# mobeets/classifying-vae-lstm

Measured on AMD Instinct MI355X. Metric: piano-roll timesteps/sec (train), higher is better.
Workload: dtype f32; 1 GPU; cfg3: cl_vrnn batch 256/GPU x seq_len 128, latent 2, 10 classes, 88-dim piano-roll, Adam-WN, hipGraph=True; global_batch=256, seq_len=128, parallelism=dp1

## Files before the change

### classifying-vae-lstm_amd/_lib.py

```python
import ctypes as C
import os

_HERE = os.path.dirname(os.path.abspath(__file__))
LIB_PATH = os.environ.get("CLV_LIB") or os.path.join(_HERE, "libclvae_hip.so")

ABI_VERSION = 600
ACT_NONE, ACT_RELU, ACT_SIGMOID, ACT_MASKPOS = 0, 1, 2, 3
GATE_HARD_SIGMOID, GATE_SIGMOID = 0, 1

_f = C.c_float
_i = C.c_int
_p = C.c_void_p
_sz = C.c_size_t
_i64 = C.c_int64
_u64 = C.c_uint64
_u32 = C.c_uint32
_d = C.c_double


class VaeStepOpts(C.Structure):
    _fields_ = [("draw", _i), ("stream_w", _u32), ("stream_z", _u32), ("step", _u32),
                ("noise_seed", _u64), ("first_w", _u64), ("first_z", _u64),
                ("step_dev", _p), ("loss_means", _p), ("bump_iterations", _p), ("bf16", _i)]

# ... 56 lines not shown


class SkinnyProduct(C.Structure):
    _fields_ = [("A", C.c_void_p), ("lda", C.c_int), ("rows", C.c_int), ("B", C.c_void_p), ("ldb", C.c_int),
                ("N", C.c_int), ("K", C.c_int), ("C", C.c_void_p), ("ldc", C.c_int), ("bias_row", C.c_void_p)]


class LabelBwdRider(C.Structure):
    _fields_ = [("D", C.c_int), ("C", C.c_int), ("Kenc_w", C.c_void_p), ("Kdec_w", C.c_void_p), ("wargs", C.c_void_p),
                ("eps", C.c_void_p), ("onehot", C.c_void_p), ("W", C.c_void_p), ("hW", C.c_void_p), ("Ka", C.c_void_p),
                ("prior_logvar", C.c_float), ("class_weight", C.c_float), ("w_kl_weight", C.c_float), ("inv_b", C.c_float),
                ("dwargs", C.c_void_p), ("dhW", C.c_void_p), ("dKa", C.c_void_p), ("dba", C.c_void_p),
                ("ws", C.c_void_p), ("ws_bytes", C.c_size_t), ("job", C.c_void_p)]


class ProfRecord(C.Structure):
    _fields_ = [("name", C.c_char * 48), ("launches", C.c_int32), ("total_ms", C.c_float)]


def _args(kind, names):
    return [kind] * len(names.split())


_VRNN_GENERATE = _args(_i, "N S nsteps D H L C gate_act z_prior") + [_u64] + _args(_p, "x_seed w")
_VAE_GENERATE = _args(_i, "N nsteps D H L C use_x_prev z_prior") + [_u64] + _args(_p, "x_seed w")
_VARY = _args(_i, "N T D H L C gate_act|use_x_prev hist_source") + [_u64] + _args(_p, "sources x0 w_enc w_dec")
_DECODE = _args(_i, "N T D H L C gate_act|use_x_prev") + [_u64] + _args(_p, "z_in x0 history w_dec noise_rows")
_VRNN_ENC, _VRNN_DEC = _args(_p, "Kx_enc Kw_enc b_enc U_enc Wz bz"), _args(_p, "Kx_dec Kz Kw_dec b_dec U_dec Wo bo")
_VAE_ENC, _VAE_DEC = _args(_p, "Kh bh Kz bz"), _args(_p, "Kd bd Ko bo")
_TEMPER = [_p, _f, _f]
_OUT, _OUT_Z = _args(_p, "Xs xhat stream"), _args(_p, "Xs xhat zout stream")
_RESUME = [_u32] + _args(_p, "state_in state_out")

SIGNATURES = {
    "clv_version": (_i, []),
    "clv_device_count": (_i, []),
    "clv_error_string": (C.c_char_p, [_i]),
    "clv_gemm_auto_split": (_i, [_i, _i, _i]),
    "clv_gemm_workspace_bytes": (_sz, [_i, _i, _i]),
    "clv_gemm_f32": (_i, [_i, _i, _i, _i, _i, _f, _p, _i, _p, _i, _f, _p, _i, _p, _i, _p, _i, _p, _sz, _p, _p]),
    "clv_gemm_grouped_tn": (_i, [_p, _i, _i, _i, _p, _i, _f, _i, _p, _sz, _p, _p]),
    "clv_splitk_reduce_multi": (_i, [_p, _i, _p, _p, _p, _i, _p, _p, _i, _p]),
    "clv_splitk_reduce_multi_outer_supported": (_i, [_i, _i, _i, _i, _i]),
    "clv_splitk_reduce_multi_outer": (_i, [_p, _i, _p, _p, _p, _i, _p, _p, _i,
                                           _i, _i, _i, _p, _i, _i, _p, _i, _p, _i, _p, _p, _i, _p, _p, _p]),
    "clv_lstm_wgrad_supported": (_i, [_i, _i, _i, _i, _i]),
    "clv_lstm_wgrad_workspace_bytes": (_sz, [_i, _i, _i, _i, _i, _i]),
    "clv_lstm_wgrad_pair_supported": (_i, [_p, _p]),
    "clv_lstm_wgrad_pair_workspace_bytes": (_sz, [_i, _i, _i, _i, _i, _i]),
    "clv_lstm_wgrad_pair": (_i, [_p, _p, _i, _p, _p, _p]),
    "clv_lstm_wgrad": (_i, [_i, _i, _p, _i, _i, _i, _p, _i, _i, _i, _i, _p, _i, _i, _p, _i, _p, _i, _p, _i, _p, _i, _f,
                               _i, _p, _sz, _p, _p]),
    "clv_gemm_grouped_tn_small2": (_i, [_p, _i, _p, _p, _i, _p, _i, _i, _i, _p]),
    "clv_gemm_grouped_auto_split": (_i, [_p, _i, _i, _i]),
    "clv_gemm_grouped_workspace_bytes": (_sz, [_p, _i, _i, _i]),
    "clv_colsum_workspace_bytes": (_sz, [_i, _i]),
    "clv_colsum_f32": (_i, [_i, _i, _p, _i, _f, _p, _p, _sz, _p]),
    "clv_lstm_seq_fwd": (_i, [_i, _i, _i, _i, _p, _p, _p, _p, _p, _p, _p, _p, _p, _p, _p]),
    "clv_lstm_seq_bwd_z": (_i, [_i, _i, _i, _i, _p, _p, _p, _p, _p, _p, _p, _i, _p, _i, _p]),
    "clv_lstm_seq_bwd": (_i, [_i, _i, _i, _i, _p, _p, _p, _p, _p, _p, _p]),
    "clv_lstm_mx_supported": (_i, [_i, _i, _i, _i]),
    "clv_lstm_mx_fwd": (_i, [_i, _i, _i, _i, _p, _i, _i, _i, _p, _p, _i, _i, _p, _p, _p, _p, _p, _p, _p]),
    "clv_lstm_mx_bwd": (_i, [_i, _i, _i, _p, _p, _p, _p, _p, _p, _i, _p, _i, _p]),
    "clv_lstm_pair_supported": (_i, [_i, _i]),
    "clv_lstm_pair_pack_floats": (_sz, []),
    "clv_lstm_pair_pack": (_i, [_i, _i, _p, _p, _p, _p, _p, _p]),
    "clv_lstm_pair_fwd": (_i, [_i, _i, _i, _i, _i, _p, _p, _p, _i, _p, _p, _p, _p, _p, _p, _p, _p, _p, _p, _i, _p, _p, _p, _p, _p,
                               _p, _p]),
    "clv_lstm_pair_bwd": (_i, [_i, _i, _i, _i, _i, _f] + [_p] * 12 + [_p, _p, _p, _p, _sz, _p, _p, _p]),
    "clv_lstm_pair_bwd_workspace_bytes": (_sz, [_i, _i, _i]),
    "clv_sparse_proj_supported": (_i, [_i, _i]),
    "clv_sparse_proj_lds_bytes": (_sz, [_i, _i]),
    "clv_sparse_proj": (_i, [_i, _i, _i, _p, _i, _i, _p, _p, _i, _p]),
    "clv_sparse_proj2": (_i, [_i, _i, _i, _i, _i, _p, _i, _p, _p, _i, _p, _i, _p, _p, _p]),
    "clv_sparse_dense_supported": (_i, [_i]),
    "clv_sparse_dense": (_i, [_i, _i, _i, _p, _i, _p, _p, _i, _p, _i, _p]),
    "clv_sparse_outer": (_i, [_i, _i, _i, _p, _i, _p, _i, _p, _i, _p, _p, _i, _p, _p, _p]),
    "clv_dense_outer_bf16_supported": (_i, [_i, _i, _i, _i, _i]),
    "clv_dense_outer_bf16": (_i, [_i, _i, _i, _p, _i, _i, _p, _i, _p, _i, _p, _p, _i, _p, _p, _p]),
    "clv_gemm_bce_f32": (_i, [_i, _i, _i, _p, _i, _p, _i, _p, _p, _i, _f, _p, _p, _i, _p, _p]),
    "clv_out_head_train_supported": (_i, [_i, _i]),
    "clv_out_head_train_workspace_bytes": (_sz, [_i]),
    "clv_out_head_train": (_i, [_i, _i, _i, _p, _p, _p, _p, _i, _i, _f, _p, _p, _p, _p, _p, _p, _p, _sz, _p, _p]),
    "clv_latent_head_supported": (_i, [_i, _i]),
    "clv_latent_head_bwd_workspace_bytes": (_sz, [_i, _i]),
    "clv_latent_head_fwd": (_i, [_i, _i, _i, _p, _p, _p, _p, _p, _p, _i, _p, _p, _p]),
    "clv_latent_head_bwd": (_i, [_i, _i, _i, _p, _p, _p, _p, _p, _i, _f, _p, _p, _p, _p, _p, _sz, _p, _p]),
    "clv_vrnn_generate_supported": (_i, [_i, _i, _i, _i]),
    "clv_vrnn_generate": (_i, _VRNN_GENERATE + _VRNN_ENC + _VRNN_DEC + _OUT),
    "clv_vae_generate_supported": (_i, [_i, _i, _i, _i]),
    "clv_vae_generate": (_i, _VAE_GENERATE + _VAE_ENC + _VAE_DEC + _OUT),
    "clv_vrnn_generate_clamped": (_i, _VRNN_GENERATE + _VRNN_ENC + _VRNN_DEC + _args(_p, "clamp") + _OUT),
    "clv_vae_generate_clamped": (_i, _VAE_GENERATE + _VAE_ENC + _VAE_DEC + _args(_p, "clamp") + _OUT),
    "clv_vrnn_generate_tempered": (_i, _VRNN_GENERATE + _VRNN_ENC + _VRNN_DEC + _TEMPER + _OUT),
    "clv_vae_generate_tempered": (_i, _VAE_GENERATE + _VAE_ENC + _VAE_DEC + _TEMPER + _OUT),
    "clv_vrnn_vary": (_i, _VARY + _VRNN_ENC + _VRNN_DEC + _TEMPER + _OUT),
    "clv_vae_vary": (_i, _VARY + _VAE_ENC + _VAE_DEC + _TEMPER + _OUT),
    "clv_take_frame": (_i, [_i64, _i, _i, _p, _p, _p, _p]),
    "clv_vrnn_vary_latents": (_i, _VARY + _VRNN_ENC + _VRNN_DEC + _TEMPER + _OUT_Z),
    "clv_vae_vary_latents": (_i, _VARY + _VAE_ENC + _VAE_DEC + _TEMPER + _OUT_Z),
    "clv_vrnn_decode": (_i, _DECODE + _VRNN_DEC + _TEMPER[:2] + _OUT),
    "clv_vae_decode": (_i, _DECODE + _VAE_DEC + _TEMPER[:2] + _OUT),
    "clv_vrnn_generate_resume": (_i, _VRNN_GENERATE + _VRNN_ENC + _VRNN_DEC + _TEMPER + _RESUME + _OUT),
    "clv_vae_generate_resume": (_i, _VAE_GENERATE[:-2] + _args(_p, "w") + _VAE_ENC + _VAE_DEC + _TEMPER + _RESUME + _OUT),
    "clv_lerp_rows": (_i, [_i64, _i64] + [_p] * 7),
    "clv_sigmoid_temper": (_i, [_i64, _p, _f, _p]),
    "clv_scale_temper": (_i, [_i64, _p, _f, _p]),
    "clv_label_fwd": (_i, [_i, _i, _p, _p, _i, _p, _p, _f, _p, _p, _p]),
    "clv_label_bwd": (_i, [_i, _i, _p, _p, _i, _p, _p, _p, _p, _f, _f, _f, _f, _p, _p, _i, _p]),
    "clv_vae_fused_supported": (_i, [_i, _i, _i, _i, _i]),
    "clv_vae_fused_workspace_bytes": (_sz, [_i, _i, _i, _i, _i, _i, _i]),
    "clv_vae_fused_step": (_i, [_i, _i, _i, _i, _i, _i, _i, _p, _p, _p, _p, _p, _p, _p, _p, _p, C.c_long, _f, _f, _f, _f, _i,
                                _p, _p, _sz, _p, _p, _p, _p, _p, _p, _p, _p, _p]),
    "clv_vrnn_label_fwd": (_i, [_i, _i, _i, _i, _p, _p, _p, _p, _p, _f, _p, _p, _p, _p, _p, _p, _p, _p, _p, _p]),
    "clv_vrnn_label_fwd_x": (_i, [_i, _i, _i, _i, _p, _i, _i, _p, _p, _p, _p, _p, _p, _p, _p, _f, _p, _p, _p, _p, _p, _p, _p, _p, _p,
                                  _p, _p, _p, _p]),
    "clv_vrnn_label_fwd_x_proj_supported": (_i, [_i, _i, _i, _i, _i]),
    "clv_vrnn_label_fwd_parts": (_i, [_i, _i, _i, _i, _p, _i, _p, _p, _p, _p, _p, _p, _f, _p, _p, _p, _p, _p, _p, _p, _p, _p,
                                  _p, _p, _p]),
    "clv_dense_window_fwd_bf16_supported": (_i, [_i, _i, _i, _i, _i]),
    "clv_dense_window_fwd_bf16_splits": (_i, [_i, _i]),
    "clv_dense_window_fwd_bf16_workspace_bytes": (_sz, [_i, _i, _i]),
    "clv_dense_window_fwd_bf16": (_i, [_i, _i, _i, _p, _i, _i, _p, _i, _p, _sz, _p]),
    "clv_vrnn_label_bwd_workspace_bytes": (_sz, [_i, _i, _i]),
    "clv_vrnn_label_bwd": (_i, [_i, _i, _i, _i, _p, _p, _p, _p, _p, _p, _p, _p, _p, _p, _f, _f, _f, _f, _p, _p, _p, _p, _p, _sz,
                                   _p, _p]),
    "clv_gauss_fwd": (_i, [_i, _i, _p, _p, _p, _i, _p, _p]),
    "clv_gauss_bwd": (_i, [_i, _i, _p, _p, _p, _i, _f, _p, _p]),
    "clv_bernoulli_nll": (_i, [_i, _i, _p, _p, _i, _f, _p, _p, _p]),
    "clv_loss_sums": (_i, [_p, _i, _i, _p, _i, _i, _p, _i, _i, _p, _i, _i, _p, _i, _i, _p, _p]),
    "clv_sum_strided": (_i, [_i, _p, _i, _f, _p, _p]),
    "clv_act_grad": (_i, [_i64, _i, _p, _p, _p, _p]),
    "clv_axpy": (_i, [_i64, _f, _p, _p, _p]),
    "clv_gather_rows": (_i, [_i64, _i64, _p, _p, _p, _i64, _i64, _p]),
    "clv_adam_wn_plan_bytes": (_sz, [_p, _i]),
    "clv_adam_wn_plan_build": (_i, [_p, _i, _p]),
    "clv_adam_wn_workspace_bytes": (_sz, [_p, _i]),
    "clv_adam_wn_step": (_i, [_p, _i, _p, _p, _p, _p, _p, _p, _p, _p, _p, _i, _f, _f, _f, _f, _i, _p, _p, _sz, _p]),
    "clv_philox_normal2": (_i, [_p, _i64, _u32, _u64, _p, _i64, _u32, _u64, _u64, _u32, _p, _p]),
    "clv_gather_rows_multi": (_i, [_i64, _p, _i64, _i, _p, _p, _p, _p, _p, _p, _p, _p, _p, _p, _p, _p]),
    "clv_philox_normal": (_i, [_p, _i64, _u64, _u32, _p, _u32, _u64, _p]),
    "clv_philox_uniform": (_i, [_p, _i64, _u64, _u32, _p, _u32, _u64, _p]),
    "clv_i32_add": (_i, [_p, C.c_int32, _p]),
    "clv_iw_accumulate": (_i, [_i, _i, _i, _i, _p, _p, _p, _p, _p, _f, _i, _p, _p, _p]),
    "clv_iw_finish": (_i, [_i, _i, _i, _p, _p, _p, _p, _p]),
    "clv_smc_sample": (_i, [_i, _i, _i, _i, _i, _p, _p, _p, _p, _p, _p, _p, _p]),
    "clv_smc_resample": (_i, [_i, _i, _i, _i, _u64, _i64, _d] + [_p] * 9),
    "clv_smc_gather": (_i, [_i, _i, _i, _i, _i, _p, _p, _p, _p, _p, _p, _p]),
    "clv_smc_backtrack": (_i, [_i, _i, _i, _i, _i, _u64, _i64, _i, _p, _p, _p, _p, _p, _p]),
    "clv_smc_init_w": (_i, [_i, _i, _i, _i, _u64, _i64, _p, _p, _p, _p, _p]),
    "clv_smc_w_posterior": (_i, [_i, _i, _i, _i, _i, _p, _p, _p, _p, _p]),
    "clv_smc_take_w": (_i, [_i, _i, _i, _i, _p, _p, _p, _p]),
    "clv_key_track_windows": (_i, [_i, _i, _i, _i, _i, _i, _i, _p, _p, _p, _p, _p, _p, _p, _u64, _i64, _p, _p, _p]),
    "clv_key_track_smooth": (_i, [_i, _i, _p, _p, _p, _p, _d, _p, _p, _p, _p, _p]),
    "clv_bernoulli_sample": (_i, [_i64, _p, _p, _p, _p]),
    "clv_bernoulli_sample_clamped": (_i, [_i64, _i, _i, _i, _p, _p, _p, _p, _p, _p]),
    "clv_dropout_rows": (_i, [_i, _i, _i, _p, _i, _p, _i, _f, _f, _p, _i, _p]),
    "clv_graph_begin_capture": (_i, [_p]),
    "clv_graph_end_capture": (_i, [_p, C.POINTER(_p)]),
    "clv_graph_launch": (_i, [_p, _p]),
    "clv_graph_destroy": (_i, [_p]),
    "clv_prof_enable": (_i, [_i]),
    "clv_prof_collect": (_i, [C.POINTER(ProfRecord), _i]),
    "clv_prof_empty_scope": (_i, [_p]),
}

_lib = None


class ClvError(RuntimeError):
    pass


def lib():
    global _lib
    if _lib is None:
        if not os.path.exists(LIB_PATH):
            raise ClvError(
                "libclvae_hip.so is not built (%s). Run `python __graft_entry__.py` or "
                "`make -C classifying-vae-lstm_amd/csrc`. There is no CPU fallback." % LIB_PATH)
        import torch
        h = C.CDLL(LIB_PATH)
        for name, (res, args) in SIGNATURES.items():
            fn = getattr(h, name)
            fn.restype = res
            fn.argtypes = args
        if h.clv_version() != ABI_VERSION:
            raise ClvError("libclvae_hip.so has ABI version %d, this binding was written for %d (include/clvae.h: "
                           "CLV_ABI_VERSION); rebuild with `make -C classifying-vae-lstm_amd/csrc`"
                           % (h.clv_version(), ABI_VERSION))
        _lib = h
    return _lib


def require_gpu():
    n = lib().clv_device_count()
    if n <= 0:
        raise ClvError("no gfx950 (MI355X) device visible; the HIP path has no CPU fallback")
    return n


def check(code, what=""):
# ... 4 lines not shown
```

### classifying-vae-lstm_amd/csrc/label_head.hip

```cpp
#include "common.h"
#include "lstm_pair_pack.h"
#include "philox.h"
#include "reduce_job.h"
#include "label_bwd_row.h"

namespace clv {

struct LabelFwdArgs {
  int B, D, C, G4;
  const float* hW;
  __device__ float* hW_out() const { return const_cast<float*>(hW); }
  const float* Ka;
  const float* ba;
  float* eps;
  struct { int on; uint32_t k0, k1, stream, step; uint64_t first; const int32_t* step_dev; } noise;
  const float* onehot;
  float prior;
  const float* Kenc_w;
  const float* benc;
  const float* Kdec_w;
  const float* bdec;
  float* wargs;
  float* W;
  float* rowloss;
  float* rb_enc;
  float* rb_dec;
};

template <int NT>
__device__ __forceinline__ void label_fwd_row(const LabelFwdArgs& a, int b, int tid, const float* s_h, float* s_wargs, float* s_w,
                                              long long oh_row = -1) {
  const int C1 = a.C - 1, NA = 2 * C1;
  __shared__ float s_eps[LH_MAXC], s_oh[LH_MAXC];
  if (tid >= NT - 64 && tid - (NT - 64) < a.C) {
    const int j = tid - (NT - 64);
    float e = 0.f;
    if (j < C1) {
      if (a.noise.on) {
        e = philox_normal_at(a.noise.first + (uint64_t)b * C1 + j, a.noise.k0, a.noise.k1, a.noise.stream,
                             a.noise.step + (a.noise.step_dev ? (uint32_t)*a.noise.step_dev : 0u));
        a.eps[(size_t)b * C1 + j] = e;
      } else {
        e = a.eps[(size_t)b * C1 + j];
      }
    }
    s_eps[j] = e;
    s_oh[j] = a.onehot ? a.onehot[(size_t)(oh_row < 0 ? b : oh_row) * a.C + j] : 0.f;
  }
  {
    __shared__ float s_part[16][2 * LH_MAXC];
    constexpr int KSL = NT / 64 < 16 ? NT / 64 : 16;
    const int col = tid & 63, sl = tid >> 6;
    if (sl < KSL) {
      float kv[(128 + KSL - 1) / KSL];
      const int cc = min(col, NA - 1);
#pragma unroll
      for (int i = 0; i < (128 + KSL - 1) / KSL; ++i) kv[i] = a.Ka[(size_t)min(sl + KSL * i, a.D - 1) * NA + cc];
      float acc = 0.f;
#pragma unroll
      for (int i = 0; i < (128 + KSL - 1) / KSL; ++i) acc = fmaf(sl + KSL * i < a.D ? s_h[sl + KSL * i] : 0.f, kv[i], acc);
      if (col < NA) s_part[sl][col] = acc;
    }
    __syncthreads();
    if (tid < NA) {
      float acc = a.ba[tid];
#pragma unroll
      for (int i = 0; i < KSL; ++i) acc += s_part[i][tid];
      s_wargs[tid] = acc;
      a.wargs[(size_t)b * NA + tid] = acc;
    }
  }
  __syncthreads();
  if (tid == 0) {
    float e[LH_MAXC];
    float S = 1.f, klw = 0.f;
    const float ep = __expf(a.prior);
    for (int j = 0; j < C1; ++j) {
      const float m = s_wargs[j], lv = s_wargs[C1 + j];
      const float sd = expf(0.5f * lv);
      e[j] = expf(m + sd * s_eps[j]);
      S += e[j];
      klw += 1.f - a.prior + lv - sd * sd / ep - m * m / ep;
    }
    e[C1] = 1.f;
    const float invS = 1.f / S;
    float qs = 0.f, wbest = -1.f, tbest = -1.f;
    int amax = 0, tmax = 0;
    for (int j = 0; j < a.C; ++j) {
      const float w = e[j] * invS;
      s_w[j] = w;
      a.W[(size_t)b * a.C + j] = w;
      qs += w + LW2;
      if (w > wbest) { wbest = w; amax = j; }
      const float tj = s_oh[j];
      if (tj > tbest) { tbest = tj; tmax = j; }
    }
    float wrec = 0.f;
    if (a.onehot)
      for (int j = 0; j < a.C; ++j) {
        const float n = (s_w[j] + LW2) / qs;
        wrec -= s_oh[j] * logf(fminf(fmaxf(n, LEPS_K), 1.f - LEPS_K));
      }
    a.rowloss[(size_t)b * 3 + 0] = -0.5f * klw;
    a.rowloss[(size_t)b * 3 + 1] = (float)C1 * wrec;
    a.rowloss[(size_t)b * 3 + 2] = (a.onehot && amax == tmax) ? 1.f : 0.f;
  }
  __syncthreads();
  for (int c = tid; c < a.G4; c += NT) {
    float e = a.benc[c], d = a.bdec[c];
    for (int j0 = 0; j0 < a.C; j0 += 8) {
      float ke[8], kd[8];
#pragma unroll
      for (int q = 0; q < 8; ++q) {
        const int j = min(j0 + q, a.C - 1);
        ke[q] = a.Kenc_w[(size_t)j * a.G4 + c];
        kd[q] = a.Kdec_w[(size_t)j * a.G4 + c];
      }
#pragma unroll
      for (int q = 0; q < 8; ++q) {
        const float w = j0 + q < a.C ? s_w[j0 + q] : 0.f;
        e = fmaf(w, ke[q], e);
        d = fmaf(w, kd[q], d);
      }
    }
    a.rb_enc[(size_t)b * a.G4 + c] = e;
    a.rb_dec[(size_t)b * a.G4 + c] = d;
  }
}

__global__ __launch_bounds__(LH_T) void vrnn_label_fwd_kernel(LabelFwdArgs a) {
  __shared__ float s_h[128], s_wargs[2 * LH_MAXC], s_w[LH_MAXC];
  const int b = blockIdx.x, tid = threadIdx.x;
  if (tid < a.D) s_h[tid] = a.hW[(size_t)b * a.D + tid];
  __syncthreads();
  label_fwd_row<LH_T>(a, b, tid, s_h, s_wargs, s_w);
}

struct LabelFwdXArgs {
  LabelFwdArgs l;
  const float* X;
  const float* Kh;
  const float* bh;
  int nx, ldx;
  PairPackArgs pack;
  const float* part; int splits;
  struct Stage {
    int on;
    const unsigned char* cur; const unsigned char* hist;
    long long cur_stride, cur_offset, hist_stride, hist_offset, row0;
    const long long* cur_table; const long long* hist_table; const long long* idx;
    const int* step_dev; int step0, period; long long cur_s, cur_o;
    float* X; float* Xh; int hist_chunk; long long hist_ld;
    const float* w_src; float* w_out;
    unsigned char* X8; unsigned char* Xh8;
  } stage;
};
__device__ __forceinline__ void label_fwd_x_block(const LabelFwdXArgs& ax, const int b, float2 (*part)[64], float* s_h, float* s_wargs,
                                                  float* s_w) {
  const LabelFwdArgs& a = ax.l;
  const int tid = threadIdx.x, lane = tid & 63;
  if (ax.pack.out) {
    for (int i = b * 1024 + tid; i < PK_TOTAL; i += a.B * 1024)
      ax.pack.out[i] = pair_pack_element(i, ax.pack.L, ax.pack.U_e, ax.pack.U_d, ax.pack.Kz, ax.pack.Wz,
                                         [](const float* p) { return *p; });
  }
  const int wave = __builtin_amdgcn_readfirstlane(tid >> 6);
  const int n2 = a.D / 2;
  const int lc = min(lane, n2 - 1);
  const float2* K2 = reinterpret_cast<const float2*>(ax.Kh);
  const float* xr = ax.X + (size_t)b * ax.ldx;
  const unsigned char* xbytes = nullptr;
  long long oh_row = -1;
  if (ax.stage.on) {
    const LabelFwdXArgs::Stage& g = ax.stage;
    long long base = 0;
    if (g.step_dev) {
      int j = (*g.step_dev - g.step0) % g.period;
      j = j < 0 ? j + g.period : j;
      base = (long long)j * g.cur_s + g.cur_o;
    }
    const long long sr = g.idx ? g.idx[base + b] : g.row0 + base + b;
    oh_row = sr;
    xbytes = g.cur + (g.cur_table ? g.cur_table[sr] : sr) * g.cur_stride + g.cur_offset;
    const unsigned char* hb = g.hist ? g.hist + (g.hist_table ? g.hist_table[sr] : sr) * g.hist_stride + g.hist_offset : nullptr;
    if (g.X8) {
      unsigned* xo8 = reinterpret_cast<unsigned*>(g.X8 + (size_t)b * ax.nx);
      unsigned* ho8 = reinterpret_cast<unsigned*>(g.Xh8 + (size_t)b * ax.nx);
      for (int c = 4 * tid; c < ax.nx; c += 4 * 1024) {
        xo8[c >> 2] = *reinterpret_cast<const unsigned*>(xbytes + c);
        if (hb) ho8[c >> 2] = *reinterpret_cast<const unsigned*>(hb + c);
      }
    } else {
      float* xo = g.X + (size_t)b * ax.ldx;
      for (int c = 4 * tid; c < ax.nx; c += 4 * 1024) {
        const unsigned v = *reinterpret_cast<const unsigned*>(xbytes + c);
        *reinterpret_cast<float4*>(xo + c) = make_float4((float)(v & 255u), (float)((v >> 8) & 255u), (float)((v >> 16) & 255u), (float)(v >> 24));
      }
      if (hb) {
        const int pieces = ax.nx / g.hist_chunk;
        for (int c = 4 * tid; c < ax.nx; c += 4 * 1024) {
          const unsigned v = *reinterpret_cast<const unsigned*>(hb + c);
          const int p = c / g.hist_chunk, w = c - p * g.hist_chunk;
          *reinterpret_cast<float4*>(g.Xh + ((size_t)b * pieces + p) * g.hist_ld + w) =
              make_float4((float)(v & 255u), (float)((v >> 8) & 255u), (float)((v >> 16) & 255u), (float)(v >> 24));
        }
      }
    }
    if (g.w_out && tid < a.C) g.w_out[(size_t)b * a.C + tid] = g.w_src[(size_t)sr * a.C + tid];
  }
  float2 acc = make_float2(0.f, 0.f);
  const int nchunk = (ax.nx + 63) / 64;
  typedef const __attribute__((address_space(1))) unsigned* gwords;
  auto xload = [&](int ch) -> unsigned {
    const int i = min(min(ch, nchunk - 1) * 64 + lane, ax.nx - 1);
    return xbytes ? ((gwords)xbytes)[i >> 2] : __builtin_bit_cast(unsigned, xr[i]);
  };
  const int xsh = 8 * (lane & 3);
  auto xval = [&](unsigned raw) { return xbytes ? (float)((raw >> xsh) & 0xffu) : __builtin_bit_cast(float, raw); };
  unsigned xa = xload(wave), xb = xload(wave + 16);
  for (int ch = wave; ch < nchunk; ch += 32) {
    const float x0 = xval(xa), x1 = xval(xb);
    const int j0 = ch * 64, j1 = (ch + 16) * 64;
    xa = xload(ch + 32); xb = xload(ch + 48);
    unsigned long long m0 = __ballot(j0 + lane < ax.nx && x0 != 0.f);
    unsigned long long m1 = __ballot(ch + 16 < nchunk && j1 + lane < ax.nx && x1 != 0.f);
    while (m0 | m1) {
      int kk[8];
      float vv[8];
#pragma unroll
      for (int q = 0; q < 8; ++q) {
        unsigned long long& m = q < 4 ? m0 : m1;
        const bool on = m != 0;
        const int bit = on ? __builtin_ctzll(m) : 0;
        m = on ? (m & (m - 1)) : 0;
        kk[q] = (q < 4 ? j0 : j1) + bit;
        const float v = __builtin_bit_cast(float, __builtin_amdgcn_readlane(__builtin_bit_cast(int, q < 4 ? x0 : x1), bit));
        vv[q] = on ? v : 0.f;
      }
      float2 kr[8];
#pragma unroll
      for (int q = 0; q < 8; ++q) kr[q] = K2[(size_t)min(kk[q], ax.nx - 1) * n2 + lc];
#pragma unroll
      for (int q = 0; q < 8; ++q) { acc.x = fmaf(vv[q], kr[q].x, acc.x); acc.y = fmaf(vv[q], kr[q].y, acc.y); }
    }
  }
  part[wave][lane] = acc;
  __syncthreads();
  if (wave == 0 && lane < n2) {
    float2 t = make_float2(ax.bh[2 * lane], ax.bh[2 * lane + 1]);
#pragma unroll
    for (int w = 0; w < 16; ++w) { t.x += part[w][lane].x; t.y += part[w][lane].y; }
    t.x = fmaxf(t.x, 0.f); t.y = fmaxf(t.y, 0.f);
    s_h[2 * lane] = t.x; s_h[2 * lane + 1] = t.y;
    float* op = a.hW_out() + (size_t)b * a.D + 2 * lane;
    op[0] = t.x; op[1] = t.y;
  }
  __syncthreads();
  label_fwd_row<1024>(a, b, tid, s_h, s_wargs, s_w, oh_row);
}

__global__ __launch_bounds__(1024) void vrnn_label_fwd_x_kernel(LabelFwdXArgs ax) {
  __shared__ float2 part[16][64];
  __shared__ float s_h[128], s_wargs[2 * LH_MAXC], s_w[LH_MAXC];
  label_fwd_x_block(ax, (int)blockIdx.x, part, s_h, s_wargs, s_w);
}

constexpr int FP_RMAX = 64;
constexpr int FP_NC = 4;
#ifndef FP_PF
#define FP_PF 4
#endif
#ifndef FP_ROUND
#define FP_ROUND 1
#endif
#ifndef FP_ABL
#define FP_ABL 0
#endif
typedef unsigned u32x4_t __attribute__((ext_vector_type(4)));
struct FrameProjArgs {
  int T, N, ldo, wgs, nset;
  const float* K[2];
  float* out[2];
};

#ifdef FRONT_STAMPS
__device__ unsigned long long g_front_wg[2048][6];
#define FRONT_STAMP(k)                                                                                               \
  do {                                                                                                               \
    __syncthreads();                                                                                                 \
    if (threadIdx.x == 0 && blockIdx.x < 2048) {                                                                     \
      unsigned long long t__;                                                                                        \
      unsigned hw__, xcc__;                                                                                          \
      asm volatile("s_memrealtime %0\n\ts_waitcnt lgkmcnt(0)" : "=s"(t__));                                          \
      asm volatile("s_getreg_b32 %0, hwreg(HW_REG_HW_ID)" : "=s"(hw__));                                             \
      asm volatile("s_getreg_b32 %0, hwreg(HW_REG_XCC_ID)" : "=s"(xcc__));                                           \
      g_front_wg[blockIdx.x][k < 2 ? k : k + 2] = t__;                                                                \
      g_front_wg[blockIdx.x][2] = hw__; g_front_wg[blockIdx.x][3] = xcc__;                                           \
    }                                                                                                                \
  } while (0)
#else
#define FRONT_STAMP(k)
#endif

__device__ __forceinline__ void frame_proj_block(const LabelFwdXArgs& ax, const FrameProjArgs& fp, const int u, float* Kl,
                                                 const unsigned char** rowp) {
  const LabelFwdXArgs::Stage& g = ax.stage;
  const int tid = threadIdx.x, lane = tid & 63;
  const int wave = __builtin_amdgcn_readfirstlane(tid >> 6);
  const int grp = u / fp.wgs, w = u - grp * fp.wgs;
  const bool second = grp >= 2;
  const int nf = ax.l.D, B = ax.l.B;
  const int nch = fp.N / 2, c0 = (grp & 1) * nch;
  const float* K = second ? fp.K[1] : fp.K[0];
  float* out = second ? fp.out[1] : fp.out[0];
  {
    const int q4 = nch / 4, nv = nf * q4;
    float4* dst = reinterpret_cast<float4*>(Kl);
    for (int i0 = tid; i0 < nv; i0 += 4 * 1024) {
      float4 v[4];
#pragma unroll
      for (int q = 0; q < 4; ++q) {
        const int e = min(i0 + q * 1024, nv - 1), k = e / q4;
        v[q] = *reinterpret_cast<const float4*>(K + (size_t)k * fp.N + c0 + 4 * (e - k * q4));
      }
#pragma unroll
      for (int q = 0; q < 4; ++q)
        if (i0 + q * 1024 < nv) dst[i0 + q * 1024] = v[q];
    }
  }
  const int nrows = w < B ? (B - w + fp.wgs - 1) / fp.wgs : 0;
  if (tid < nrows) {
    const int b = w + tid * fp.wgs;
    long long base = 0;
    if (g.step_dev) {
      int j = (*g.step_dev - g.step0) % g.period;
      j = j < 0 ? j + g.period : j;
      base = (long long)j * g.cur_s + g.cur_o;
    }
    const long long sr = g.idx ? g.idx[base + b] : g.row0 + base + b;
    rowp[tid] = second ? g.hist + (g.hist_table ? g.hist_table[sr] : sr) * g.hist_stride + g.hist_offset
                       : g.cur + (g.cur_table ? g.cur_table[sr] : sr) * g.cur_stride + g.cur_offset;
  }
  __syncthreads();
  FRONT_STAMP(2);
  const int nq = nrows * fp.T;
  if (nq == 0) return;
  const int colb = min(lane, nch / 4 - 1) * 4;
// ... 19 lines not shown
  auto advance_a = [&]() {
    ta += 16;
    if (ta >= fp.T) {
      do { ta -= fp.T; ++ra; } while (ta >= fp.T);
      base_a = rowbase(ra);
    }
  };
  const unsigned so_step = 16u * (unsigned)fp.ldo * 4u, so_wrap = (unsigned)(fp.wgs - 1) * (unsigned)fp.T * (unsigned)fp.ldo * 4u;
  unsigned so = (unsigned)(((w + ri * fp.wgs) * fp.T + t) * fp.ldo + c0) * 4u;
  auto advance_c = [&]() {
    t += 16; so += so_step;
    while (t >= fp.T) { t -= fp.T; so += so_wrap; }
  };
  unsigned qx0[FP_PF], qx1[FP_PF];
#pragma unroll
  for (int j = 0; j < FP_PF; ++j) {
    const bool ok = wave + 16 * j < nq;
    frame(ok ? base_a : base0, ok ? ta : 0, qx0[j], qx1[j]);
    __builtin_amdgcn_raw_buffer_store_b128(u32x4_t{0u, 0u, 0u, 0u}, r_out, (int)0x80000000u, 0, 0);
    advance_a();
  }
  for (int qb = wave; qb < nq; qb += 16 * FP_PF) {
#pragma unroll
    for (int j = 0; j < FP_PF; ++j) {
      const int q = qb + 16 * j;
      const bool live = q < nq;
      const float fx0 = (float)((qx0[j] >> sh0) & 0xffu), fx1 = (float)((qx1[j] >> sh1) & 0xffu);
      const bool more = q + 16 * FP_PF < nq;
      if (FP_ABL != 3) frame(more ? base_a : base0, more ? ta : 0, qx0[j], qx1[j]);
      advance_a();
      unsigned long long m0 = __ballot(live && v0 && fx0 != 0.f), m1 = __ballot(live && v1 && fx1 != 0.f);
      float acc[FP_NC];
#pragma unroll
      for (int c = 0; c < FP_NC; ++c) acc[c] = 0.f;
      auto rounds = [&](unsigned long long m, const float fx, const int kbase) {
        if (FP_ROUND == 1) {
          while (m) {
            const int k = __builtin_ctzll(m);
            asm("s_bitset0_b64 %0, %1" : "+s"(m) : "s"(k));
            const float v = __builtin_bit_cast(float, __builtin_amdgcn_readlane(__builtin_bit_cast(int, fx), k));
            const float4 k4 = *reinterpret_cast<const float4*>(Kl + (kbase + k) * nch + colb);
            acc[0] = fmaf(v, k4.x, acc[0]); acc[1] = fmaf(v, k4.y, acc[1]); acc[2] = fmaf(v, k4.z, acc[2]); acc[3] = fmaf(v, k4.w, acc[3]);
          }
          return;
        }
        while (m) {
          float v[FP_ROUND], kv[FP_ROUND][FP_NC];
          bool on[FP_ROUND];
#pragma unroll
          for (int r = 0; r < FP_ROUND; ++r) {
            on[r] = m != 0;
            const int k = on[r] ? __builtin_ctzll(m) : 0;
            m &= m - 1;
            v[r] = __builtin_bit_cast(float, __builtin_amdgcn_readlane(__builtin_bit_cast(int, fx), k));
            const float4 k4 = *reinterpret_cast<const float4*>(Kl + (kbase + k) * nch + colb);
            kv[r][0] = k4.x; kv[r][1] = k4.y; kv[r][2] = k4.z; kv[r][3] = k4.w;
          }
#pragma unroll
          for (int r = 0; r < FP_ROUND; ++r)
#pragma unroll
            for (int c = 0; c < FP_NC; ++c) acc[c] = (r == 0 || on[r]) ? fmaf(v[r], kv[r][c], acc[c]) : acc[c];
        }
      };
      if (FP_ABL != 2) {
        rounds(m0, fx0, 0);
        rounds(m1, fx1, 64);
      } else {
        acc[0] = fx0; acc[1] = fx1;
      }
      __builtin_amdgcn_raw_buffer_store_b128(u32x4_t{__builtin_bit_cast(unsigned, acc[0]), __builtin_bit_cast(unsigned, acc[1]),
                                                      __builtin_bit_cast(unsigned, acc[2]), __builtin_bit_cast(unsigned, acc[3])},
                                             r_out, (int)((live && FP_ABL != 1) ? vo : 0x80000000u), (int)so, 0);
      advance_c();
    }
  }
}

__global__ __launch_bounds__(1024) __attribute__((amdgpu_num_sgpr(72))) void vrnn_front_kernel(LabelFwdXArgs ax, FrameProjArgs fp) {
  __shared__ float2 part[16][64];
  __shared__ float s_h[128], s_wargs[2 * LH_MAXC], s_w[LH_MAXC];
  __shared__ const unsigned char* rowp[FP_RMAX];
  extern __shared__ __attribute__((aligned(16))) float fp_kl[];
  FRONT_STAMP(0);
  if ((int)blockIdx.x < ax.l.B) label_fwd_x_block(ax, (int)blockIdx.x, part, s_h, s_wargs, s_w);
  else frame_proj_block(ax, fp, (int)blockIdx.x - ax.l.B, fp_kl, rowp);
  FRONT_STAMP(1);
}

__global__ __launch_bounds__(LH_T) void vrnn_label_fwd_parts_kernel(LabelFwdXArgs ax) {
  constexpr int NWV = LH_T / 64;
  __shared__ float2 part[NWV][64];
  __shared__ float s_h[128], s_wargs[2 * LH_MAXC], s_w[LH_MAXC];
  const LabelFwdArgs& a = ax.l;
  const int tid = threadIdx.x, lane = tid & 63;
  if (ax.pack.out) {
    for (int i = blockIdx.x * LH_T + tid; i < PK_TOTAL; i += gridDim.x * LH_T)
      ax.pack.out[i] = pair_pack_element(i, ax.pack.L, ax.pack.U_e, ax.pack.U_d, ax.pack.Kz, ax.pack.Wz,
                                         [](const float* p) { return *p; });
  }
  const int wave = __builtin_amdgcn_readfirstlane(tid >> 6);
  const int b = blockIdx.x;
  const int n2 = a.D / 2;
  const int lc = min(lane, n2 - 1);
  float2 acc = make_float2(0.f, 0.f);
  const float2* pp = reinterpret_cast<const float2*>(ax.part + (size_t)b * a.D) + lc;
  const size_t cs = (size_t)a.B * a.D / 2;
  for (int c0 = wave; c0 < ax.splits; c0 += 8 * NWV) {
    float2 v[8];
#pragma unroll
    for (int q = 0; q < 8; ++q) v[q] = pp[(size_t)min(c0 + NWV * q, ax.splits - 1) * cs];
#pragma unroll
    for (int q = 0; q < 8; ++q) {
      const float mk = c0 + NWV * q < ax.splits ? 1.f : 0.f;
      acc.x = fmaf(v[q].x, mk, acc.x); acc.y = fmaf(v[q].y, mk, acc.y);
    }
  }
  part[wave][lane] = acc;
  __syncthreads();
  if (wave == 0 && lane < n2) {
    float2 t = make_float2(ax.bh[2 * lane], ax.bh[2 * lane + 1]);
#pragma unroll
    for (int w = 0; w < NWV; ++w) { t.x += part[w][lane].x; t.y += part[w][lane].y; }
    t.x = fmaxf(t.x, 0.f); t.y = fmaxf(t.y, 0.f);
    s_h[2 * lane] = t.x; s_h[2 * lane + 1] = t.y;
    float* op = a.hW_out() + (size_t)b * a.D + 2 * lane;
    op[0] = t.x; op[1] = t.y;
  }
  __syncthreads();
  label_fwd_row<LH_T>(a, b, tid, s_h, s_wargs, s_w);
}

__global__ __launch_bounds__(LH_T) void vrnn_label_bwd_kernel(LabelBwdArgs a) {
  label_bwd_row<LH_T>(a, (int)blockIdx.x, (int)threadIdx.x);
}

}

using namespace clv;

extern "C" int clv_vrnn_label_fwd(int B, int D, int C, int G4, const float* hW, const float* Ka, const float* ba,
                                  const float* eps, const float* onehot, float prior_logvar,
                                  const float* Kenc_w, const float* benc, const float* Kdec_w, const float* bdec,
                                  float* wargs, float* W, float* rowloss, float* rb_enc, float* rb_dec, void* stream) {
  if (B <= 0 || D <= 0 || D > 128 || C < 2 || C > LH_MAXC || G4 <= 0) return CLV_EINVAL;
  if (!hW || !Ka || !ba || !eps || !Kenc_w || !benc || !Kdec_w || !bdec || !wargs || !W || !rowloss || !rb_enc || !rb_dec)
    return CLV_EINVAL;
  LabelFwdArgs a{B, D, C, G4, hW, Ka, ba, const_cast<float*>(eps), {0, 0, 0, 0, 0, 0, nullptr}, onehot, prior_logvar, Kenc_w, benc,
                 Kdec_w, bdec, wargs, W, rowloss, rb_enc, rb_dec};
  hipStream_t s = (hipStream_t)stream;
  ProfScope p("vrnn_label_fwd", s);
  hipLaunchKernelGGL(vrnn_label_fwd_kernel, dim3(B), dim3(LH_T), 0, s, a);
  return launch_status();
}

extern "C" size_t clv_vrnn_label_bwd_workspace_bytes(int B, int D, int C) {
  return (size_t)B * (D + 1) * 2 * (C - 1) * sizeof(float);
}

extern "C" int clv_vrnn_label_bwd(int B, int D, int C, int G4, const float* dzsum_enc, const float* dzsum_dec,
                                     const float* Kenc_w, const float* Kdec_w, const float* wargs, const float* eps,
                                     const float* onehot, const float* W, const float* hW, const float* Ka,
                                     float prior_logvar, float class_weight, float w_kl_weight, float inv_b,
                                     float* dwargs, float* dhW, float* dKa, float* dba, void* ws, size_t ws_bytes,
                                     clv_reduce_job* job, void* stream) {
  if (job) memset(job, 0, sizeof(*job));
  if (B <= 0 || D <= 0 || D > 128 || C < 2 || C > LH_MAXC || G4 <= 0) return CLV_EINVAL;
  if (!dzsum_enc || !dzsum_dec || !Kenc_w || !Kdec_w || !wargs || !eps || !onehot || !W || !hW || !Ka || !dwargs || !dhW)
    return CLV_EINVAL;
  const bool wg = dKa != nullptr;
  if (wg && (!dba || !ws || ws_bytes < clv_vrnn_label_bwd_workspace_bytes(B, D, C))) return CLV_EWORKSPACE;
  LabelBwdArgs a{B, D, C, G4, dzsum_enc, dzsum_dec, Kenc_w, Kdec_w, wargs, eps, onehot, W, hW, Ka,
                 prior_logvar, class_weight, w_kl_weight, inv_b, dwargs, dhW, wg ? (float*)ws : nullptr};
  hipStream_t s = (hipStream_t)stream;
  {
    ProfScope p("vrnn_label_bwd", s);
    hipLaunchKernelGGL(vrnn_label_bwd_kernel, dim3(B), dim3(LH_T), 0, s, a);
  }
  int st = launch_status();
  if (st || !wg) return st;
  ReduceJob j;
  memset(&j, 0, sizeof(j));
  const int NA = 2 * (C - 1);
  j.partial = (const float*)ws;
  j.M = D + 1; j.N = NA; j.splits = B; j.nprob = 2;
  j.alpha = 1.f; j.beta = 0.f; j.act = CLV_ACT_NONE;
  j.prob[0] = ReduceProb{dKa, NA, 0};
  j.prob[1] = ReduceProb{dba, NA, D};
  if (job && B > 1) memcpy(job, &j, sizeof(j));
  else st = launch_reduce(j, s);
  return st;
}

extern "C" int clv_vrnn_label_fwd_x_proj_supported(int B, int D, int nx, int T, int N);

static int label_fwd_x_launch(int B, int D, int C, int G4, const float* X, int ldx, int nx, const float* Kh, const float* part,
                              int splits, const clv_label_stage* stage, const float* bh, float* hW_out, const float* Ka, const float* ba,
                              float* eps, const float* onehot, float prior_logvar,
                              const float* Kenc_w, const float* benc, const float* Kdec_w, const float* bdec,
                              float* wargs, float* W, float* rowloss, float* rb_enc, float* rb_dec,
                              const clv_noise_draw* noise, const clv_pair_pack_src* pack, const clv_frame_proj* proj, void* stream) {
  if (pack && (pack->H != LH || !clv_lstm_pair_supported(pack->H, pack->L) || !pack->U_enc || !pack->U_dec || !pack->Kz ||
               !pack->Wz || !pack->pack || ((uintptr_t)pack->pack) % 16))
    return CLV_EINVAL;
  if (B <= 0 || D <= 0 || D > 128 || D % 2 != 0 || C < 2 || C > LH_MAXC || G4 <= 0) return CLV_EINVAL;
  if (part ? (splits <= 0 || ((uintptr_t)part) % 8 != 0)
           : (nx <= 0 || ldx < nx || (!X && !(stage && stage->X8)) || !Kh || ((uintptr_t)Kh) % 8 != 0)) return CLV_EINVAL;
  if (stage) {
    const clv_label_stage& g = *stage;
    if (part || !g.cur || nx % 4 || ldx % 4 || ((uintptr_t)g.cur) % 4 || g.cur_stride % 4 || g.cur_offset % 4) return CLV_EINVAL;
    if (g.hist && (((uintptr_t)g.hist) % 4 || g.hist_stride % 4 || g.hist_offset % 4)) return CLV_EINVAL;
    if (g.X8) {
      if (((uintptr_t)g.X8) % 4 || (g.hist && (!g.Xh8 || ((uintptr_t)g.Xh8) % 4))) return CLV_EINVAL;
    } else {
      if (!g.X || ((uintptr_t)g.X) % 16) return CLV_EINVAL;
      if (g.hist && (!g.Xh || g.hist_chunk <= 0 || g.hist_chunk % 4 || nx % g.hist_chunk || g.hist_ld % 4 || g.hist_ld < g.hist_chunk ||
                     ((uintptr_t)g.Xh) % 16))
        return CLV_EINVAL;
    }
    if ((g.w_out != nullptr) != (g.w_src != nullptr)) return CLV_EINVAL;
    if (g.cursor.step_dev && g.cursor.period < 1) return CLV_EINVAL;
  }
  if (!bh || !hW_out || !Ka || !ba || !eps || !Kenc_w || !benc || !Kdec_w || !bdec || !wargs || !W || !rowloss ||
      !rb_enc || !rb_dec)
    return CLV_EINVAL;
  LabelFwdXArgs a{{B, D, C, G4, hW_out, Ka, ba, eps, {0, 0, 0, 0, 0, 0, nullptr}, onehot, prior_logvar, Kenc_w, benc, Kdec_w, bdec,
                   wargs, W, rowloss, rb_enc, rb_dec}, X, Kh, bh, nx, ldx, {0, nullptr, nullptr, nullptr, nullptr, nullptr}, part, splits, {}};
  if (stage) {
    const clv_label_stage& g = *stage;
    a.stage = LabelFwdXArgs::Stage{1, g.cur, g.hist, (long long)g.cur_stride, (long long)g.cur_offset, (long long)g.hist_stride,
                                   (long long)g.hist_offset, (long long)g.row0, (const long long*)g.cur_table,
                                   (const long long*)g.hist_table, (const long long*)g.idx, g.cursor.step_dev, g.cursor.step0,
                                   g.cursor.period, (long long)g.cursor.stride, (long long)g.cursor.offset, g.X, g.Xh, g.hist_chunk,
                                   (long long)g.hist_ld, g.w_src, g.w_out, g.X8, g.Xh8};
    if (g.w_src) a.l.onehot = g.w_src;
  }
  if (pack) a.pack = PairPackArgs{pack->L, pack->U_enc, pack->U_dec, pack->Kz, pack->Wz, reinterpret_cast<float4*>(pack->pack)};
  if (noise) {
    a.l.noise.on = 1; a.l.noise.k0 = (uint32_t)noise->seed; a.l.noise.k1 = (uint32_t)(noise->seed >> 32);
    a.l.noise.stream = noise->stream; a.l.noise.step = noise->step; a.l.noise.first = noise->first;
    a.l.noise.step_dev = noise->step_dev;
  }
  hipStream_t s = (hipStream_t)stream;
  if (proj) {
    if (!clv_vrnn_label_fwd_x_proj_supported(B, D, nx, proj->T, proj->N) || !stage || !stage->X8 || part || proj->ldo < proj->N ||
        (size_t)B * proj->T * proj->ldo * 4 >= ((size_t)1 << 31) || proj->ldo % 4 || ((uintptr_t)proj->out_cur) % 16 || ((uintptr_t)proj->out_hist) % 16 ||
        !proj->K_cur || !proj->out_cur || ((uintptr_t)proj->K_cur) % 16 || (proj->K_hist && (!proj->out_hist || !stage->hist ||
        ((uintptr_t)proj->K_hist) % 16)))
      return CLV_EINVAL;
    FrameProjArgs fp;
    memset(&fp, 0, sizeof(fp));
    fp.T = proj->T; fp.N = proj->N; fp.ldo = proj->ldo; fp.nset = proj->K_hist ? 2 : 1;
    fp.K[0] = proj->K_cur; fp.out[0] = proj->out_cur; fp.K[1] = proj->K_hist; fp.out[1] = proj->out_hist;
    const int groups = 2 * fp.nset;
    int wgs = 256 / groups;
    wgs = wgs > B ? B : wgs;
    const int need = (B + FP_RMAX - 1) / FP_RMAX;
    wgs = wgs < need ? need : wgs;
    fp.wgs = wgs;
    size_t lds = (size_t)D * (proj->N / 2) * sizeof(float);
#ifdef FRONT_STAMPS
    if (const char* e = getenv("CLV_EXP_FRONT_LDS")) lds = (size_t)atoi(e);
#endif
    if (int e = clv::allow_dynamic_lds(reinterpret_cast<const void*>(vrnn_front_kernel), 64 * 1024)) return e;
    ProfScope p("vrnn_front", s);
    hipLaunchKernelGGL(vrnn_front_kernel, dim3(B + groups * wgs), dim3(1024), lds, s, a, fp);
    return launch_status();
  }
  ProfScope p("vrnn_label_fwd", s);
  if (part) hipLaunchKernelGGL(vrnn_label_fwd_parts_kernel, dim3(B), dim3(LH_T), 0, s, a);
  else hipLaunchKernelGGL(vrnn_label_fwd_x_kernel, dim3(B), dim3(1024), 0, s, a);
  return launch_status();
}

#ifdef FRONT_STAMPS
extern "C" int clv_debug_front_wg(unsigned long long* host_out) {
  return (int)hipMemcpyFromSymbol(host_out, HIP_SYMBOL(clv::g_front_wg), sizeof(unsigned long long) * 2048 * 6);
}
#endif

extern "C" int clv_vrnn_label_fwd_x_proj_supported(int B, int D, int nx, int T, int N) {
  return B >= 1 && D >= 4 && D <= 128 && D % 4 == 0 && T >= 1 && (long long)T * D == nx && N >= 8 && N % 8 == 0 && N / 2 <= 64 * clv::FP_NC &&
         (size_t)D * (N / 2) * sizeof(float) <= 64 * 1024 && (size_t)B * T * N * sizeof(float) < ((size_t)1 << 31);
}

extern "C" int clv_vrnn_label_fwd_x(int B, int D, int C, int G4, const float* X, int ldx, int nx, const float* Kh,
                                    const clv_label_stage* stage,
                                    const float* bh, float* hW_out, const float* Ka, const float* ba,
                                    float* eps, const float* onehot, float prior_logvar,
                                    const float* Kenc_w, const float* benc, const float* Kdec_w, const float* bdec,
                                    float* wargs, float* W, float* rowloss, float* rb_enc, float* rb_dec,
                                    const clv_noise_draw* noise, const clv_pair_pack_src* pack, const clv_frame_proj* proj,
                                    void* stream) {
  if (stage)
    return label_fwd_x_launch(B, D, C, G4, stage->X, ldx, nx, Kh, nullptr, 0, stage, bh, hW_out, Ka, ba, eps, stage->w_src,
                              prior_logvar, Kenc_w, benc, Kdec_w, bdec, wargs, W, rowloss, rb_enc, rb_dec, noise, pack, proj, stream);
  if (proj) return CLV_EINVAL;
  return label_fwd_x_launch(B, D, C, G4, X, ldx, nx, Kh, nullptr, 0, nullptr, bh, hW_out, Ka, ba, eps, onehot, prior_logvar, Kenc_w, benc,
                            Kdec_w, bdec, wargs, W, rowloss, rb_enc, rb_dec, noise, pack, nullptr, stream);
}

extern "C" int clv_vrnn_label_fwd_parts(int B, int D, int C, int G4, const float* part, int splits,
                                        const float* bh, float* hW_out, const float* Ka, const float* ba,
                                        float* eps, const float* onehot, float prior_logvar,
                                        const float* Kenc_w, const float* benc, const float* Kdec_w, const float* bdec,
                                        float* wargs, float* W, float* rowloss, float* rb_enc, float* rb_dec,
                                        const clv_noise_draw* noise, const clv_pair_pack_src* pack, void* stream) {
  if (!part) return CLV_EINVAL;
  return label_fwd_x_launch(B, D, C, G4, nullptr, 0, 0, nullptr, part, splits, nullptr, bh, hW_out, Ka, ba, eps, onehot, prior_logvar, Kenc_w,
                            benc, Kdec_w, bdec, wargs, W, rowloss, rb_enc, rb_dec, noise, pack, nullptr, stream);
}
```

### classifying-vae-lstm_amd/csrc/out_head.hip

```cpp
#include "out_head_args.h"
#include "reduce_job.h"

namespace clv {

typedef float f32x4 __attribute__((ext_vector_type(4)));

constexpr int OH_T = 6;
constexpr int OH_KS = OH / 4;
constexpr int OH_LD = 116;
constexpr int OH_NW = 8;
static_assert(OH_RB == 16 * OH_NW, "rows per block");
constexpr int OH_TILE = 16 * OH_LD;
constexpr int OH_P3 = 5;

#ifdef OH_STAMPS
__device__ unsigned long long g_oh_stamps[16];
#define OHS(k) do { if (blockIdx.x == 0 && threadIdx.x == 0) g_oh_stamps[k] = __builtin_readcyclecounter(); } while (0)
#else
#define OHS(k) do { } while (0)
#endif


__global__ __launch_bounds__(64 * OH_NW) void out_head_train_kernel(OutHeadArgs a) {
  extern __shared__ __attribute__((aligned(16))) float oh_lds[];
  float* WoL = oh_lds;
  float* hsT = oh_lds + OH * OH_LD;
  float* dlT = hsT + OH_NW * OH_TILE;
  const int tid = threadIdx.x, lane = tid & 63;
  const int wave = __builtin_amdgcn_readfirstlane(tid >> 6);
  const int r = lane & 15, q = lane >> 4;
  OHS(0);

  float bias[OH_T];
#pragma unroll
  for (int j = 0; j < OH_T; ++j) bias[j] = a.bo[min(16 * j + r, OH - 1)];

  const int t0 = wave < 4 ? OH_P3 * wave : 4 * OH_P3 + (OH_P3 - 1) * (wave - 4);
  const int nt = wave < 4 ? OH_P3 : OH_P3 - 1;
  int tm[OH_P3], tn[OH_P3];
  f32x4 acc3[OH_P3];
#pragma unroll
  for (int i = 0; i < OH_P3; ++i) {
    const int t = min(t0 + i, OH_T * OH_T - 1);
    tm[i] = t / OH_T; tn[i] = t - tm[i] * OH_T;
    acc3[i] = (f32x4){0.f, 0.f, 0.f, 0.f};
  }
  float* myhs = hsT + wave * OH_TILE;
  float* mydl = dlT + wave * OH_TILE;

  float4 hv[6];
  auto load_hs = [&](int row0) {
#pragma unroll
    for (int i = 0; i < 6; ++i) {
      const int e = min(lane + 64 * i, 16 * (OH / 4) - 1);
      const int rr = e / (OH / 4), c4 = e - rr * (OH / 4);
      hv[i] = *reinterpret_cast<const float4*>(a.hs + (size_t)min(row0 + rr, a.R - 1) * OH + 4 * c4);
    }
  };
  float y[OH_T][4];
  auto load_y = [&](int row0) {
#pragma unroll
    for (int j = 0; j < OH_T; ++j)
#pragma unroll
      for (int reg = 0; reg < 4; ++reg)
        y[j][reg] = static_cast<const float*>(a.Y)[(size_t)min(row0 + 4 * q + reg, a.R - 1) * a.ldy + min(16 * j + r, OH - 1)];
  };
  load_hs(blockIdx.x * OH_RB + wave * 16);
  load_y(blockIdx.x * OH_RB + wave * 16);
  {
    constexpr int NV = OH * (OH / 4);
    float4 wv[(NV + 64 * OH_NW - 1) / (64 * OH_NW)];
#pragma unroll
    for (int i = 0; i < (NV + 64 * OH_NW - 1) / (64 * OH_NW); ++i) {
      const int e = min(tid + 64 * OH_NW * i, NV - 1);
      const int h = e / (OH / 4), c4 = e - h * (OH / 4);
      wv[i] = *reinterpret_cast<const float4*>(a.Wo + h * OH + 4 * c4);
    }
#pragma unroll
    for (int i = 0; i < (NV + 64 * OH_NW - 1) / (64 * OH_NW); ++i) {
      const int e = tid + 64 * OH_NW * i;
      const int h = e / (OH / 4), c4 = e - h * (OH / 4);
      if (e < NV) *reinterpret_cast<float4*>(WoL + h * OH_LD + 4 * c4) = wv[i];
    }
// ... 102 lines not shown
#pragma unroll
          for (int j = 0; j < OH_T; ++j) bn[j] = WoL[wrow[j] + 4 * (s + 1)];
        }
        __builtin_amdgcn_sched_barrier(0);
#pragma unroll
        for (int j = 0; j < OH_T; ++j) acc[j] = __builtin_amdgcn_mfma_f32_16x16x4f32(av, bv[j], acc[j], 0, 0, 0);
        __builtin_amdgcn_sched_barrier(0);
        if (s + 1 < OH_KS) {
          av = an;
#pragma unroll
          for (int j = 0; j < OH_T; ++j) bv[j] = bn[j];
        }
      }
    }
#pragma unroll
    for (int reg = 0; reg < 4; ++reg) {
      const int row = row0 + 4 * q + reg;
#pragma unroll
      for (int j = 0; j < OH_T; ++j) {
        const int col = 16 * j + r;
        if (row < a.R && col < OH) a.dhs[(size_t)row * OH + col] = acc[j][reg];
      }
    }
    OHS(5);
    __syncthreads();
    OHS(6);

    {
      auto p3off = [&](int ks) { return (ks >> 2) * OH_TILE + ((ks & 3) * 4 + q) * OH_LD + r; };
      float av[OH_P3], bv[OH_P3];
#pragma unroll
      for (int i = 0; i < OH_P3; ++i) {
        av[i] = hsT[p3off(0) + 16 * tm[i]];
        bv[i] = dlT[p3off(0) + 16 * tn[i]];
      }
#pragma unroll 4
      for (int ks = 0; ks < OH_RB / 4; ++ks) {
        const int off = p3off(min(ks + 1, OH_RB / 4 - 1));
        float an[OH_P3], bn[OH_P3];
#pragma unroll
        for (int i = 0; i < OH_P3; ++i) {
          an[i] = hsT[off + 16 * tm[i]];
          bn[i] = dlT[off + 16 * tn[i]];
        }
        __builtin_amdgcn_sched_barrier(0);
#pragma unroll
        for (int i = 0; i < OH_P3; ++i)
          if (i < nt) acc3[i] = __builtin_amdgcn_mfma_f32_16x16x4f32(av[i], bv[i], acc3[i], 0, 0, 0);
        __builtin_amdgcn_sched_barrier(0);
#pragma unroll
        for (int i = 0; i < OH_P3; ++i) { av[i] = an[i]; bv[i] = bn[i]; }
      }
    }
    OHS(7);
    __syncthreads();
  }
  float* slab = a.partial + (size_t)blockIdx.x * OH_SLAB_ROWS * OH;
#pragma unroll
  for (int i = 0; i < OH_P3; ++i)
#pragma unroll
    for (int reg = 0; reg < 4; ++reg) {
      const int h = 16 * tm[i] + 4 * q + reg, o = 16 * tn[i] + r;
      if (i < nt && h < OH_SLAB_ROWS && o < OH) slab[h * OH + o] = acc3[i][reg];
    }
  OHS(8);
}

#ifdef OH_STAMPS
}
extern "C" int clv_debug_out_head_stamps(unsigned long long* host_out) {
  return (int)hipMemcpyFromSymbol(host_out, HIP_SYMBOL(clv::g_oh_stamps), sizeof(unsigned long long) * 16);
}
namespace clv {
#endif
static int out_head_wgs(int R) {
  const int blocks = (R + OH_RB - 1) / OH_RB;
  return blocks < 256 ? blocks : 256;
}

}

extern "C" int clv_out_head_train_supported(int H, int D) { return H == clv::OH && D == clv::OH; }

extern "C" size_t clv_out_head_train_workspace_bytes(int R) {
  return R > 0 ? (size_t)clv::out_head_wgs(R) * clv::OH_SLAB_ROWS * clv::OH * sizeof(float) : 0;
}

extern "C" int clv_out_head_train(int R, int H, int D, const float* hs, const float* Wo, const float* bo,
                                  const void* Y, int y_u8, int ldy, float scale, float* logits, float* rownll, float* dlogits,
                                  float* dhs, float* dWo, float* dbo, void* ws, size_t ws_bytes, clv_reduce_job* job,
                                  void* stream) {
  using namespace clv;
  if (!clv_out_head_train_supported(H, D) || R <= 0 || ldy < D) return CLV_EINVAL;
  if (!hs || !Wo || !bo || !Y || !rownll || !dhs || !dWo || !dbo) return CLV_EINVAL;
  if (((uintptr_t)hs) % 16 != 0 || ((uintptr_t)Wo) % 16 != 0) return CLV_EINVAL;
  if (!ws || ws_bytes < clv_out_head_train_workspace_bytes(R)) return CLV_EWORKSPACE;
  hipStream_t s = (hipStream_t)stream;
  const size_t lds = (size_t)(OH * OH_LD + 2 * OH_NW * OH_TILE) * sizeof(float);
  if (int e = clv::allow_dynamic_lds(reinterpret_cast<const void*>(out_head_train_kernel), (int)lds)) return e;
  const int wgs = out_head_wgs(R);
  OutHeadArgs a{R, ldy, scale, hs, Wo, bo, Y, y_u8 != 0, logits, rownll, dlogits, dhs, (float*)ws};
  static const bool f32_only = [] { const char* e = getenv("CLV_OUT_HEAD_F32"); return e && e[0] == '1'; }();
  if (!(f32_only && !y_u8) && out_head_bf16_ok(a)) {
    if (int e = launch_out_head_bf16(a, wgs, s)) return e;
  } else {
    if (y_u8) return CLV_EINVAL;
    ProfScope p("out_head_train", s);
    hipLaunchKernelGGL(out_head_train_kernel, dim3(wgs), dim3(64 * OH_NW), lds, s, a);
  }
  int st = launch_status();
  if (st) return st;
  ReduceJob j;
  memset(&j, 0, sizeof(j));
  j.partial = (const float*)ws; j.M = OH_SLAB_ROWS; j.N = OH; j.splits = wgs; j.nprob = 2;
  j.alpha = 1.f; j.beta = 0.f; j.act = CLV_ACT_NONE;
  j.prob[0] = ReduceProb{dWo, OH, 0};
  j.prob[1] = ReduceProb{dbo, OH, OH};
  if (job && wgs > 1) {
    memcpy(job, &j, sizeof(j));
    return CLV_OK;
  }
  if (job) memset(job, 0, sizeof(*job));
  return launch_reduce(j, s);
}
```

### classifying-vae-lstm_amd/csrc/out_head_args.h

```cpp
#pragma once
#include "common.h"

namespace clv {

constexpr int OH = 88;
constexpr int OH_SLAB_ROWS = OH + 1;
constexpr int OH_RB = 128;

struct OutHeadArgs {
  int R, ldy;
  float scale;
  const float* hs;
  const float* Wo;
  const float* bo;
  const void* Y;
  int y_u8;
  float* logits;
  float* rownll;
  float* dlogits;
  float* dhs;
  float* partial;
};

bool out_head_bf16_ok(const OutHeadArgs& a);
int launch_out_head_bf16(const OutHeadArgs& a, int wgs, hipStream_t s);

}
```

### classifying-vae-lstm_amd/csrc/out_head_bf16.hip

```cpp
#include "out_head_args.h"

namespace clv {

typedef __bf16 bf16x8 __attribute__((ext_vector_type(8)));
typedef float f32x4 __attribute__((ext_vector_type(4)));
typedef float f32x16 __attribute__((ext_vector_type(16)));
typedef unsigned u32x4 __attribute__((ext_vector_type(4)));

constexpr int OB_NW = 8;
constexpr int OB_FRAG = 1024;
constexpr int OB_IMG = 3 * 6 * 3 * OB_FRAG;
constexpr int OB_DLT = 96 * 16;
constexpr int OB_LDS = 2 * OB_IMG + OB_NW * OB_DLT * 4;
static_assert(OB_LDS <= 160 * 1024, "LDS");
static_assert(OB_NW * 18 * 64 * 16 <= OB_LDS, "the final reduction's rounds fit");

#ifdef OB_STAMPS
__device__ unsigned long long g_ob_stamps[16];
__device__ unsigned long long g_ob_wg[256][4];
#define OBW(k) do { if (threadIdx.x == 0) { unsigned long long t_; asm volatile("s_memrealtime %0\n\ts_waitcnt lgkmcnt(0)" : "=s"(t_)); g_ob_wg[blockIdx.x][k] = t_; } } while (0)
#define OBS(k) do { if (blockIdx.x == 0 && threadIdx.x == 0) g_ob_stamps[k] = __builtin_readcyclecounter(); } while (0)
#else
#define OBW(k) do { } while (0)
#define OBS(k) do { } while (0)
#endif

__device__ __forceinline__ void ob_split8(const float (&v)[8], u32x4 (&f)[3]) {
#pragma unroll
  for (int i = 0; i < 4; ++i) {
    unsigned pc[3];
#ifdef OB_SHIFT_SPLIT
    bf16_split_pair(v[2 * i], v[2 * i + 1], pc);
#else
    bf16_split_pair_dot2(v[2 * i], v[2 * i + 1], pc);
#endif
    f[0][i] = pc[0]; f[1][i] = pc[1]; f[2][i] = pc[2];
  }
}
__device__ __forceinline__ bf16x8 ob_frag(const u32x4& v) { return __builtin_bit_cast(bf16x8, v); }

typedef __amdgpu_buffer_rsrc_t ob_rsrc_t;
constexpr unsigned OB_OOB = 0x80000000u;
__device__ __forceinline__ ob_rsrc_t ob_rsrc(const void* p, size_t bytes) {
  return __builtin_amdgcn_make_buffer_rsrc(const_cast<void*>(p), 0, (int)(unsigned)bytes, 0x00020000);
}
__device__ __forceinline__ float ob_u2f(unsigned u) { return __builtin_bit_cast(float, u); }
__device__ __forceinline__ float ob_load1(ob_rsrc_t r, unsigned voff, int imm) {
  return __builtin_bit_cast(float, __builtin_amdgcn_raw_buffer_load_b32(r, (int)voff + imm, 0, 0));
}
__device__ __forceinline__ void ob_load4(ob_rsrc_t r, unsigned voff, float (&v)[4]) {
  const u32x4 x = __builtin_amdgcn_raw_buffer_load_b128(r, (int)voff, 0, 0);
#pragma unroll
  for (int i = 0; i < 4; ++i) v[i] = ob_u2f(x[i]);
}
__device__ __forceinline__ void ob_load8(ob_rsrc_t r, unsigned voff, float (&v)[8]) {
  const u32x4 x = __builtin_amdgcn_raw_buffer_load_b128(r, (int)voff, 0, 0);
  const u32x4 z = __builtin_amdgcn_raw_buffer_load_b128(r, (int)voff + 16, 0, 0);
#pragma unroll
  for (int i = 0; i < 4; ++i) { v[i] = ob_u2f(x[i]); v[4 + i] = ob_u2f(z[i]); }
}
__device__ __forceinline__ void ob_store4(const float (&v)[4], ob_rsrc_t r, unsigned voff) {
  const u32x4 x = {__builtin_bit_cast(unsigned, v[0]), __builtin_bit_cast(unsigned, v[1]), __builtin_bit_cast(unsigned, v[2]),
                   __builtin_bit_cast(unsigned, v[3])};
  __builtin_amdgcn_raw_buffer_store_b128(x, r, (int)voff, 0, 0);
}
__device__ __forceinline__ void ob_store1(float v, ob_rsrc_t r, unsigned voff) {
  __builtin_amdgcn_raw_buffer_store_b32(__builtin_bit_cast(unsigned, v), r, (int)voff, 0, 0);
}

#define OB_PROD6(MFMA, acc, A, B)                                   \
  do {                                                              \
    acc = MFMA(ob_frag(A[2]), ob_frag(B[0]), acc, 0, 0, 0);         \
    acc = MFMA(ob_frag(A[1]), ob_frag(B[1]), acc, 0, 0, 0);         \
    acc = MFMA(ob_frag(A[0]), ob_frag(B[2]), acc, 0, 0, 0);         \
    acc = MFMA(ob_frag(A[1]), ob_frag(B[0]), acc, 0, 0, 0);         \
    acc = MFMA(ob_frag(A[0]), ob_frag(B[1]), acc, 0, 0, 0);         \
    acc = MFMA(ob_frag(A[0]), ob_frag(B[0]), acc, 0, 0, 0);         \
  } while (0)

__device__ __forceinline__ int ob_dlt_line(int note) { return (((note >> 4) * 4 + (note & 3)) * 4 + ((note >> 2) & 3)) * 16; }

template <bool YU8>
__global__ __launch_bounds__(64 * OB_NW) void out_head_bf16_kernel(OutHeadArgs a) {
  extern __shared__ __attribute__((aligned(16))) char ob_lds[];
  char* A1 = ob_lds;
  char* A2 = ob_lds + OB_IMG;
  const int tid = threadIdx.x, lane = tid & 63;
  const int wave = __builtin_amdgcn_readfirstlane(tid >> 6);
  const int r = lane & 15, q = lane >> 4, n32 = lane & 31, kh = lane >> 5;
  float* dlT = reinterpret_cast<float*>(ob_lds + 2 * OB_IMG) + wave * OB_DLT;
  OBS(0);
  OBW(0);

  const ob_rsrc_t r_hs = ob_rsrc(a.hs, (size_t)a.R * OH * 4), r_y = ob_rsrc(a.Y, (size_t)a.R * a.ldy * (YU8 ? 1 : 4));
  const ob_rsrc_t r_lg = ob_rsrc(a.logits, a.logits ? (size_t)a.R * OH * 4 : 0);
  const ob_rsrc_t r_dl = ob_rsrc(a.dlogits, a.dlogits ? (size_t)a.R * OH * 4 : 0);
  const ob_rsrc_t r_dh = ob_rsrc(a.dhs, (size_t)a.R * OH * 4), r_nl = ob_rsrc(a.rownll, (size_t)a.R * 4);
  const unsigned c_off = (16 * 0 + 4 * q) * 4u;
  const bool c5 = q < 2;

  float hv[3][8];
  auto load_hv = [&](int row0) {
#pragma unroll
    for (int s = 0; s < 3; ++s)
      ob_load8(r_hs, (s == 2 && q == 3) ? OB_OOB : (unsigned)(row0 + r) * (OH * 4u) + (32 * s + 8 * q) * 4u, hv[s]);
  };
  load_hv(blockIdx.x * OH_RB + wave * 16);

  {
    const ob_rsrc_t r_wo = ob_rsrc(a.Wo, (size_t)OH * OH * 4), r_bo = ob_rsrc(a.bo, (size_t)OH * 4);
    const int m = r, qq = q;
    const unsigned l0 = (8 * qq * OH + m) * 4u;
    const unsigned l1 = (m * OH + 4 * qq) * 4u;
    float wv[5][8];
#pragma unroll
    for (int it = 0; it < 5; ++it) {
      const int F = min(8 * it + wave, 35);
      const int img = F >= 18, fr = F - 18 * img, j = fr / 3, s = fr - 3 * j;
      if (!img) {
        const unsigned vo = (16 * j + m < OH) ? l0 + (32 * s * OH + 16 * j) * 4u : OB_OOB;
#pragma unroll
        for (int e = 0; e < 8; ++e) wv[it][e] = ob_u2f(__builtin_amdgcn_raw_buffer_load_b32(r_wo, (int)vo + e * OH * 4, 0, 0));
        const float bias = ob_u2f(__builtin_amdgcn_raw_buffer_load_b32(r_bo, (s == 2 && qq == 3) ? (16 * j + m) * 4 : (int)OB_OOB, 0, 0));
        wv[it][0] = (s == 2 && qq == 3) ? bias : wv[it][0];
      } else {
        const unsigned vo = l1 + (16 * j * OH + 32 * s) * 4u;
        const u32x4 lo = __builtin_amdgcn_raw_buffer_load_b128(r_wo, (int)vo, 0, 0);
        const u32x4 hi = __builtin_amdgcn_raw_buffer_load_b128(r_wo, (s == 2 && qq >= 2) ? (int)OB_OOB : (int)vo + 64, 0, 0);
#pragma unroll
        for (int e = 0; e < 4; ++e) { wv[it][e] = ob_u2f(lo[e]); wv[it][4 + e] = ob_u2f(hi[e]); }
      }
    }
#pragma unroll
    for (int it = 0; it < 5; ++it) {
      const int F = 8 * it + wave;
      if (F < 36) {
        u32x4 f[3];
        ob_split8(wv[it], f);
        char* base = (F >= 18 ? A2 + (F - 18) * OB_FRAG : A1 + F * OB_FRAG) + lane * 16;
#pragma unroll
        for (int p = 0; p < 3; ++p) *reinterpret_cast<u32x4*>(base + p * 18 * OB_FRAG) = f[p];
      }
    }
  }

  f32x16 acc3[3][3];
#pragma unroll
  for (int i = 0; i < 3; ++i)
#pragma unroll
    for (int j = 0; j < 3; ++j)
#pragma unroll
      for (int e = 0; e < 16; ++e) acc3[i][j][e] = 0.f;
#pragma unroll
  for (int s = 0; s < 3; ++s) asm volatile("" :: "v"(hv[s][0]), "v"(hv[s][4]));
  OBS(10);
  __syncthreads();
  OBS(1);
  OBW(1);

  for (int blk = blockIdx.x; blk * OH_RB < a.R; blk += gridDim.x) {
    const int row0 = blk * OH_RB + wave * 16;
    if (row0 >= a.R) continue;
    const unsigned row = row0 + r;
    const bool rok = (int)row < a.R;
    const unsigned o_row = row * (OH * 4u) + c_off;
    const unsigned o5 = c5 ? o_row + 5 * 64 : OB_OOB;

    load_hv(row0);
    OBS(2);

    float y[6][4];
    f32x4 acc[6];
#pragma unroll
    for (int j = 0; j < 6; ++j) acc[j] = (f32x4){0.f, 0.f, 0.f, 0.f};
#pragma unroll
    for (int s = 0; s < 3; ++s) {
      if (s == 2) hv[2][0] = q == 3 ? 1.f : hv[2][0];
      u32x4 B[3];
      ob_split8(hv[s], B);
      if (s == 2) {
        __builtin_amdgcn_sched_barrier(0);
#pragma unroll
        for (int j = 0; j < 6; ++j) {
          if (YU8) y[j][0] = ob_load1(r_y, row * (unsigned)a.ldy + 4 * q + 16 * j, 0);
          else ob_load4(r_y, row * (a.ldy * 4u) + c_off + 64 * j, y[j]);
        }
        __builtin_amdgcn_sched_barrier(0);
      }
#pragma unroll
      for (int j = 0; j < 6; ++j) {
        u32x4 A[3];
#pragma unroll
// ... 76 lines not shown
    OBS(5);

    {
      f32x4 acc2[6];
#pragma unroll
      for (int j = 0; j < 6; ++j) acc2[j] = (f32x4){0.f, 0.f, 0.f, 0.f};
#pragma unroll
      for (int s = 0; s < 3; ++s) {
        const float v[8] = {acc[2 * s][0], acc[2 * s][1], acc[2 * s][2], acc[2 * s][3],
                            acc[2 * s + 1][0], acc[2 * s + 1][1], acc[2 * s + 1][2], acc[2 * s + 1][3]};
        u32x4 B[3];
        ob_split8(v, B);
#pragma unroll
        for (int j = 0; j < 6; ++j) {
          u32x4 A[3];
#pragma unroll
          for (int p = 0; p < 3; ++p) A[p] = *reinterpret_cast<const u32x4*>(A2 + ((p * 6 + j) * 3 + s) * OB_FRAG + lane * 16);
          OB_PROD6(__builtin_amdgcn_mfma_f32_16x16x32_bf16, acc2[j], A, B);
        }
      }
#pragma unroll
      for (int j = 0; j < 6; ++j) {
        const float d4[4] = {acc2[j][0], acc2[j][1], acc2[j][2], acc2[j][3]};
        ob_store4(d4, r_dh, j < 5 ? o_row + 64 * j : o5);
      }
    }
    asm volatile("" :: "v"(pf0), "v"(pf1));
    OBS(6);
  }

  OBW(2);
  float* slab = a.partial + (size_t)blockIdx.x * OH_SLAB_ROWS * OH;
  float4* red = reinterpret_cast<float4*>(ob_lds);
  __syncthreads();
#pragma unroll
  for (int half = 0; half < 2; ++half) {
#pragma unroll
    for (int ff = 0; ff < 18; ++ff) {
      const int f = 18 * half + ff, jm = f / 12, jn = (f >> 2) % 3, i4 = f & 3;
      red[(wave * 18 + ff) * 64 + lane] = make_float4(acc3[jm][jn][4 * i4], acc3[jm][jn][4 * i4 + 1], acc3[jm][jn][4 * i4 + 2],
                                                      acc3[jm][jn][4 * i4 + 3]);
    }
    __syncthreads();
#pragma unroll
    for (int k = 0; k < 3; ++k) {
      const int v = tid + 64 * OB_NW * k;
      if (v < 18 * 64) {
        const int ff = v >> 6, l = v & 63;
        float4 sum = red[ff * 64 + l];
#pragma unroll
        for (int w = 1; w < OB_NW; ++w) {
          const float4 x = red[(w * 18 + ff) * 64 + l];
          sum.x += x.x; sum.y += x.y; sum.z += x.z; sum.w += x.w;
        }
        const int f = 18 * half + ff, jm = f / 12, jn = (f >> 2) % 3, i4 = f & 3;
        const int h = 32 * jm + 8 * i4 + 4 * (l >> 5), note = 32 * jn + (l & 31);
        const float o4[4] = {sum.x, sum.y, sum.z, sum.w};
#pragma unroll
        for (int i = 0; i < 4; ++i)
          if (h + i < OH_SLAB_ROWS && note < OH) slab[(h + i) * OH + note] = o4[i];
      }
    }
    if (half == 0) __syncthreads();
  }
  OBS(7);
  OBW(3);
}

#ifdef OB_STAMPS
}
extern "C" int clv_debug_out_head_bf16_stamps(unsigned long long* host_out) {
  return (int)hipMemcpyFromSymbol(host_out, HIP_SYMBOL(clv::g_ob_stamps), sizeof(unsigned long long) * 16);
}
extern "C" int clv_debug_out_head_bf16_wg(unsigned long long* host_out) {
  return (int)hipMemcpyFromSymbol(host_out, HIP_SYMBOL(clv::g_ob_wg), sizeof(unsigned long long) * 1024);
}
namespace clv {
#endif

bool out_head_bf16_ok(const OutHeadArgs& a) {
  auto al = [](const void* p) { return ((uintptr_t)p) % 16 == 0; };
  const size_t widest = (size_t)a.R * (size_t)(a.ldy > OH ? a.ldy : OH) * 4;
  const bool y_ok = a.y_u8 ? (((uintptr_t)a.Y) % 4 == 0) : al(a.Y);
  return widest < 0x80000000ull && al(a.hs) && y_ok && a.ldy % 4 == 0 && al(a.dhs) && al(a.logits) && al(a.dlogits);
}

int launch_out_head_bf16(const OutHeadArgs& a, int wgs, hipStream_t s) {
  ProfScope p("out_head_bf16", s);
  if (a.y_u8) {
    if (int e = allow_dynamic_lds(reinterpret_cast<const void*>(out_head_bf16_kernel<true>), OB_LDS)) return e;
    hipLaunchKernelGGL(out_head_bf16_kernel<true>, dim3(wgs), dim3(64 * OB_NW), OB_LDS, s, a);
  } else {
    if (int e = allow_dynamic_lds(reinterpret_cast<const void*>(out_head_bf16_kernel<false>), OB_LDS)) return e;
    hipLaunchKernelGGL(out_head_bf16_kernel<false>, dim3(wgs), dim3(64 * OB_NW), OB_LDS, s, a);
  }
  return CLV_OK;
}

}
```

### classifying-vae-lstm_amd/engine.py

```python
import contextlib
import ctypes as C
import os
import warnings

import numpy as np
import torch

from . import _lib, ops
from .engine_dropout import VrnnDropout
from .engine_generate import VaeGenerate, VrnnGenerate
from .ops import ACT_MASKPOS, ACT_NONE, ACT_RELU, ACT_SIGMOID
from .params import FlatParams, fuse_heads


def vae_param_shapes(cfg):
    D, H, L, Hc, Cn = cfg['D'], cfg['H'], cfg['L'], cfg['Hc'], cfg['C']
    dec_in = Cn + (D if cfg['use_x_prev'] else 0) + L
    head = [('h_w/kernel', (D, Hc)), ('h_w/bias', (Hc,)),
            ('w_mean/kernel', (Hc, Cn - 1)), ('w_mean/bias', (Cn - 1,)),
            ('w_log_var/kernel', (Hc, Cn - 1)), ('w_log_var/bias', (Cn - 1,))]
    if H > 0:
        return head + [('h/kernel', (D + Cn, H)), ('h/bias', (H,)),
                       ('z_mean/kernel', (H, L)), ('z_mean/bias', (L,)),
                       ('z_log_var/kernel', (H, L)), ('z_log_var/bias', (L,)),
                       ('decoder_h/kernel', (dec_in, H)), ('decoder_h/bias', (H,)),
                       ('x_decoded_mean/kernel', (H, D)), ('x_decoded_mean/bias', (D,))]
    return head + [('z_mean/kernel', (D + Cn, L)), ('z_mean/bias', (L,)),
                   ('z_log_var/kernel', (D + Cn, L)), ('z_log_var/bias', (L,)),
                   ('x_decoded_mean/kernel', (dec_in, D)), ('x_decoded_mean/bias', (D,))]


def vrnn_param_shapes(cfg):
    D, H, L, T, Cn = cfg['D'], cfg['H'], cfg['L'], cfg['T'], cfg['C']
    dec_in = (D if cfg['use_x_prev'] else 0) + L + Cn
    return [('hW/kernel', (T * D, D)), ('hW/bias', (D,)),
            ('Wargs/kernel', (D, 2 * (Cn - 1))), ('Wargs/bias', (2 * (Cn - 1),)),
            ('encoder_h/kernel', (D + Cn, 4 * H)), ('encoder_h/recurrent_kernel', (H, 4 * H)),
            ('encoder_h/bias', (4 * H,)),
            ('Z_mean/kernel', (H, L)), ('Z_mean/bias', (L,)),
            ('Z_log_var/kernel', (H, L)), ('Z_log_var/bias', (L,)),
            ('decoder_h/kernel', (dec_in, 4 * H)), ('decoder_h/recurrent_kernel', (H, 4 * H)),
            ('decoder_h/bias', (4 * H,)),
            ('X_decoded_mean/kernel', (H, D)), ('X_decoded_mean/bias', (D,))]


SWITCHES = {
    'fuse_pair':      (None,                   True,  "the separate sequence kernels (csrc/lstm.hip) instead of encoder + latent head + decoder as one launch"),
    'sparse_inputs':  (None,                   True,  "dense GEMM input projections instead of row gathers of the notes that are on"),
    'keep_logits':    (None,                   True,  "the fused output head does not store its logits (what a replayed training step does: 11.5 / 92 MB per step)"),
    'fuse_head':      ('CLV_FUSE_HEAD',        True,  "output head as GEMM + NLL + three backward GEMMs instead of one launch"),
    'bf16_wgrad':     ('CLV_BF16_WGRAD',       True,  "the LSTM kernel gradients on the f32 MFMA GEMM instead of split-bf16 products"),
    'wgrad_pair':     ('CLV_WGRAD_PAIR',       True,  "one kernel-gradient launch per LSTM instead of both in one"),
    'dense_hw_grad':  ('CLV_DENSE_HW_GRAD',    True,  "the hW kernel gradient by walking the notes instead of dense on the bf16 matrix cores"),
    'dense_hw_fwd':   ('CLV_DENSE_HW_FWD',     True,  "the hW forward product by walking the notes at every batch size"),
    'label_in_pair':  ('CLV_LABEL_IN_PAIR',    True,  "the label path's backward as a launch of its own instead of the pair backward kernel's epilogue"),
    'fuse_latent':    ('CLV_FUSE_LATENT',      True,  "the latent head as GEMM + pointwise launches instead of csrc/latent_head.hip"),
    'lstm_mx':        ('CLV_USE_MX',           True,  "large batches on the generic chain instead of csrc/lstm_mx.hip"),
    'frames_u8':      ('CLV_FRAMES_U8',        True,  "the large-batch step widens its byte batch to float (rounds 4-5) instead of reading bytes"),
    'front_fused':    ('CLV_FRONT_FUSED',      True,  "the frame projections as a launch of their own behind the label launch instead of workgroups of it (csrc/label_head.hip: vrnn_front_kernel)"),
    'tail_launch':    ('CLV_TAIL_LAUNCH',      True,  "the hW kernel gradient as a launch of its own in front of grads_tail() instead of workgroups of the reduction launch that ends it (csrc/tail_launch.hip)"),
    'fine_grid':      ('CLV_FINE_GRID',        False, "twice the workgroups, half the rows each, for the LSTM kernel gradients (what tune_dp_schedule may pick next to an all-reduce)"),
    'fuse_notes':     ('CLV_FUSE_NOTES',       False, "input projections gathered inside the pair forward from note lists (+48 us on MI355X: profiles/r03_notes_fusion_ab.txt)"),
}


def switch(cfg, key):
    env, default, _ = SWITCHES[key]
    if key in cfg:
        return bool(cfg[key])
    if env is not None and env in os.environ:
        return os.environ[env] != '0'
    return default


def _f(device, *shape):
    return torch.empty(*shape, dtype=torch.float32, device=device)


class _EngineBase:
    def __init__(self, cfg, batch_size, shapes, device, head_pairs=(), grads_pre=0):
        _lib.require_gpu()
        self.cfg = dict(cfg)
        self.B = int(batch_size)
        self.device = torch.device(device)
        phys, aliases = fuse_heads(shapes, head_pairs)
        self.P = FlatParams(shapes, self.device, phys, aliases, pre=grads_pre)
        self.ws = ops.Workspace(self.device, 8 << 20)
        self.ws2 = ops.Workspace(self.device, 8 << 20)
        self.rq = ops.ReduceQueue(self.device)
        self.side = torch.cuda.Stream(device=self.device) if cfg.get('two_streams', False) else None
        self.scal = torch.zeros(8, dtype=torch.float32, device=self.device)
        self.kl_weight = float(cfg.get('kl_weight', 1.0))
        self.w_kl_weight = float(cfg.get('w_kl_weight', 1.0))
        self.class_weight = float(cfg.get('class_weight', 1.0))

    def losses(self):
        s = self.scal.detach().cpu().numpy().astype(np.float64)
        out = dict(vae=s[0], kl_z=s[1], kl_w=s[2], w_rec=s[3], acc=s[4])
        out['total'] = (out['vae'] + self.w_kl_weight * out['kl_w'] + self.class_weight * out['w_rec']
                        + self.kl_weight * out['kl_z'])
        out['elbo'] = -(out['vae'] + out['kl_z'] + out['kl_w'] + out['w_rec'])
        return out

    def _mean_into(self, n, x, stride, slot):
        ops.sum_strided(n, x, stride, 1.0 / n, self.scal[slot:])

    def _side(self):
        if self.side is None:
            return contextlib.nullcontext()
        self.side.wait_stream(torch.cuda.current_stream())
        return torch.cuda.stream(self.side)

    def _side_more(self):
        return contextlib.nullcontext() if self.side is None else torch.cuda.stream(self.side)

    def _join(self):
        if self.side is not None:
            torch.cuda.current_stream().wait_stream(self.side)


class VaeEngine(VaeGenerate, _EngineBase):

    def __init__(self, cfg, batch_size, device='cuda:0'):
        super().__init__(cfg, batch_size, vae_param_shapes(cfg), device,
                         head_pairs=[('w_mean', 'w_log_var', 'wargs'), ('z_mean', 'z_log_var', 'zargs')])
        B, D, H, L, Hc, Cn = self.B, cfg['D'], cfg['H'], cfg['L'], cfg['Hc'], cfg['C']
        d = self.device
        self.xoff = D if cfg['use_x_prev'] else 0
        L_ = _lib.lib()
        self.fused = H > 0 and bool(cfg.get('fused_step', True)) and bool(L_.clv_vae_fused_supported(D, H, Hc, Cn, L))
        self.stage_spec = None
        names = ['h_w', 'wargs', 'h', 'zargs', 'decoder_h', 'x_decoded_mean']
        self._offs = (C.c_int64 * 12)(*[self.P.offsets.get('%s/%s' % (n, w), 0) for n in names for w in ('kernel', 'bias')])
        ws_bytes = L_.clv_vae_fused_workspace_bytes(B, D, H, Hc, Cn, L, int(cfg['use_x_prev'])) if self.fused else 0
        self._fused_ws = torch.empty(max(ws_bytes, 16), dtype=torch.uint8, device=self.device) if self.fused else None
        self.h_w = _f(d, B, Hc)
        self.wargs = _f(d, B, 2 * (Cn - 1))
        self.w = _f(d, B, Cn)
        self.rowloss = _f(d, B, 3)
        self.h = _f(d, B, max(H, 1))
        self.zargs = _f(d, B, 2 * L)
        self.z = _f(d, B, L)
        self.h_dec = _f(d, B, max(H, 1))
# ... 119 lines not shown
            return
        g, ws, xo = ops.gemm, self.ws, self.xoff
        if H == 0:
            return self._grads_without_hidden_layers(x, xp, w_true, eps_w, eps_z, inv)
        g(self.h_dec, self.dlogits, P.g('x_decoded_mean/kernel'), H, D, B, ta=True, ws=ws)
        ops.colsum(self.dlogits, B, D, P.g('x_decoded_mean/bias'), ws)
        g(self.dlogits, P.p('x_decoded_mean/kernel'), self.d_hdec, B, H, D, tb=True, act=ACT_MASKPOS, aux=self.h_dec,
          ws=ws)
        g(self.w, self.d_hdec, P.g('decoder_h/kernel'), Cn, H, B, ta=True, ws=ws)
        if cfg['use_x_prev']:
            g(xp, self.d_hdec, P.rows(P.grads, 'decoder_h/kernel', Cn), D, H, B, ta=True, ws=ws)
        g(self.z, self.d_hdec, P.rows(P.grads, 'decoder_h/kernel', Cn + xo), L, H, B, ta=True, ws=ws)
        ops.colsum(self.d_hdec, B, H, P.g('decoder_h/bias'), ws)
        g(self.d_hdec, P.p('decoder_h/kernel'), self.dw, B, Cn, H, tb=True, ws=ws)
        g(self.d_hdec, P.rows(P.params, 'decoder_h/kernel', Cn + xo), self.dz, B, L, H, tb=True, ws=ws)
        ops.gauss_bwd(B, L, self.zargs, eps_z, self.dz, L, self.kl_weight * inv, self.dzargs)
        g(self.h, self.dzargs, P.g('zargs/kernel'), H, 2 * L, B, ta=True, ws=ws)
        ops.colsum(self.dzargs, B, 2 * L, P.g('zargs/bias'), ws)
        g(self.dzargs, P.p('zargs/kernel'), self.d_h, B, H, 2 * L, tb=True, act=ACT_MASKPOS, aux=self.h, ws=ws)
        g(x, self.d_h, P.g('h/kernel'), D, H, B, ta=True, ws=ws)
        g(self.w, self.d_h, P.rows(P.grads, 'h/kernel', D), Cn, H, B, ta=True, ws=ws)
        ops.colsum(self.d_h, B, H, P.g('h/bias'), ws)
        g(self.d_h, P.rows(P.params, 'h/kernel', D), self.dw, B, Cn, H, tb=True, beta=1.0, ws=ws)
        self._label_head_grads(x, w_true, eps_w, inv)


    def _label_head_grads(self, x, w_true, eps_w, inv):
        cfg, P, B = self.cfg, self.P, self.B
        D, Hc, Cn = cfg['D'], cfg['Hc'], cfg['C']
        C1, g, ws = Cn - 1, ops.gemm, self.ws
        ops.label_bwd(B, Cn, self.wargs, self.wargs[:, C1:], 2 * C1, eps_w, w_true, self.w, self.dw,
                      cfg['w_log_var_prior'], self.class_weight, self.w_kl_weight, inv,
                      self.dwargs, self.dwargs[:, C1:], 2 * C1)
        g(self.h_w, self.dwargs, P.g('wargs/kernel'), Hc, 2 * C1, B, ta=True, ws=ws)
        ops.colsum(self.dwargs, B, 2 * C1, P.g('wargs/bias'), ws)
        g(self.dwargs, P.p('wargs/kernel'), self.d_hw, B, Hc, 2 * C1, tb=True, act=ACT_MASKPOS, aux=self.h_w, ws=ws)
        g(x, self.d_hw, P.g('h_w/kernel'), D, Hc, B, ta=True, ws=ws)
        ops.colsum(self.d_hw, B, Hc, P.g('h_w/bias'), ws)

    def _grads_without_hidden_layers(self, x, xp, w_true, eps_w, eps_z, inv):
        cfg, P, B = self.cfg, self.P, self.B
        D, L, Cn = cfg['D'], cfg['L'], cfg['C']
        g, ws, xo, K = ops.gemm, self.ws, self.xoff, 'x_decoded_mean/kernel'
        g(self.w, self.dlogits, P.g(K), Cn, D, B, ta=True, ws=ws)
        if cfg['use_x_prev']:
            g(xp, self.dlogits, P.rows(P.grads, K, Cn), D, D, B, ta=True, ws=ws)
        g(self.z, self.dlogits, P.rows(P.grads, K, Cn + xo), L, D, B, ta=True, ws=ws)
        ops.colsum(self.dlogits, B, D, P.g('x_decoded_mean/bias'), ws)
        g(self.dlogits, P.p(K), self.dw, B, Cn, D, tb=True, ws=ws)
        g(self.dlogits, P.rows(P.params, K, Cn + xo), self.dz, B, L, D, tb=True, ws=ws)
        ops.gauss_bwd(B, L, self.zargs, eps_z, self.dz, L, self.kl_weight * inv, self.dzargs)
        g(x, self.dzargs, P.g('zargs/kernel'), D, 2 * L, B, ta=True, ws=ws)
        g(self.w, self.dzargs, P.rows(P.grads, 'zargs/kernel', D), Cn, 2 * L, B, ta=True, ws=ws)
        ops.colsum(self.dzargs, B, 2 * L, P.g('zargs/bias'), ws)
        g(self.dzargs, P.rows(P.params, 'zargs/kernel', D), self.dw, B, Cn, 2 * L, tb=True, beta=1.0, ws=ws)
        self._label_head_grads(x, w_true, eps_w, inv)


class VrnnEngine(VrnnDropout, VrnnGenerate, _EngineBase):

    def __init__(self, cfg, batch_size, device='cuda:0'):
        super().__init__(cfg, batch_size, vrnn_param_shapes(cfg), device,
                         head_pairs=[('Z_mean', 'Z_log_var', 'Zargs')], grads_pre=cfg['D'])
        B, D, H, L, T, Cn = self.B, cfg['D'], cfg['H'], cfg['L'], cfg['T'], cfg['C']
        d = self.device
        BT = B * T
        if H != 88:
            warnings.warn("cl_vrnn with %d LSTM units runs on the generic kernels (csrc/lstm_any.hip, GEMM heads): several times "
                          "slower per step than the default 88 units, which the fused kernels are laid out for" % H, stacklevel=2)
        self.gate_act = _lib.GATE_HARD_SIGMOID if cfg.get('gate_act', 'hard_sigmoid') == 'hard_sigmoid' \
            else _lib.GATE_SIGMOID
        self.off = D if cfg['use_x_prev'] else 0
        self.dropout = float(cfg.get('dropout', 0.0) or 0.0)
        if not 0.0 <= self.dropout < 1.0:
            raise ValueError("dropout must be in [0, 1)")
        self._train_pass = False
        sw = lambda key: switch(cfg, key)
        self.fuse_pair = sw('fuse_pair') and ops.lstm_pair_supported(L, H) and not self.dropout
        self.fine_grid = sw('fine_grid')
        self.pair_pack = _f(d, ops.lstm_pair_pack_floats()) if self.fuse_pair else None
        self.sparse_inputs = sw('sparse_inputs') and ops.sparse_proj_supported(D, 4 * H)
        self.fuse_head = sw('fuse_head') and ops.out_head_train_supported(H, D)
        self._head_done = False
        self.keep_logits = sw('keep_logits')
        self.bf16_wgrad = sw('bf16_wgrad')
        self.frames_exact_bf16 = bool(cfg.get('frames_exact_bf16', False))
        self.wgrad_pair = sw('wgrad_pair')
        self.dense_hw_grad = sw('dense_hw_grad')
        self.dense_hw_fwd = sw('dense_hw_fwd') and B >= int(os.environ.get('CLV_DENSE_HW_FWD_ROWS', '512'))
        self.ws_hw = None
        self.stage_spec = None
        self._f8 = None
        self.ws_b = None
        self.label_in_pair = sw('label_in_pair') and self.fuse_pair
        self.fuse_latent = sw('fuse_latent') and ops.latent_head_supported(H, L)
        self.use_mx = sw('lstm_mx') and not self.fuse_pair and not self.dropout and self.sparse_inputs \
            and ops.lstm_mx_supported(B, D, L, H)
        self.frames_u8 = sw('frames_u8')
        self.front_fused = sw('front_fused')
        self.tail_launch = sw('tail_launch')
        self.halves_adjacent = False
        self._hw_outer = None
        self.fuse_notes = sw('fuse_notes') and self.fuse_pair and self.sparse_inputs and D == ops.NOTE_NONE
        self.notes_valid = False
        if self.fuse_notes:
            self.notes_enc = torch.full((BT, ops.NOTE_ROW), ops.NOTE_NONE, dtype=torch.uint8, device=d)
            self.notes_dec = torch.full((BT, ops.NOTE_ROW), ops.NOTE_NONE, dtype=torch.uint8, device=d)
        self.hW = _f(d, B, D)
        self.wargs = _f(d, B, 2 * (Cn - 1))
        self.W = _f(d, B, Cn)
        self.rowloss = _f(d, B, 3)
        self.wk_enc = _f(d, B, 4 * H)
        self.wk_dec = _f(d, B, 4 * H)
        self.gates_enc = _f(d, BT, 4 * H)
        self.gates_dec = _f(d, BT, 4 * H)
        aux2 = self.fuse_pair or self.use_mx
        self.hs_enc, self.cs_enc = _f(d, BT, H), _f(d, BT, 2 * H if aux2 else H)
        self.hs_dec, self.cs_dec = _f(d, BT, H), _f(d, BT, 2 * H if aux2 else H)
        self.zargs = _f(d, BT, 2 * L)
        self.xz_ld = (self.off + L + 3) // 4 * 4
        self.XZ = torch.zeros(BT, self.xz_ld, dtype=torch.float32, device=d)
        self.Z = self.XZ[:, self.off:self.off + L]
        self.rowkl = _f(d, BT)
        self.klterm = _f(d, BT, L)
        self.logits = _f(d, BT, D)
        self.dlogits = _f(d, BT, D)
        self.rownll = _f(d, BT)
        self.dhs = _f(d, BT, H)
        self.dzsum_enc, self.dzsum_dec = _f(d, B, 4 * H), _f(d, B, 4 * H)
        self.dZ = _f(d, BT, L)
        self.dzargs = _f(d, BT, 2 * L)
        self.dW = _f(d, B, Cn)
        self.dwargs = _f(d, B, 2 * (Cn - 1))
        self.dhW = _f(d, B, D)
        self.gdot = self.P.grads_pre[:D] if (self.P.grads_pre.numel() >= D and self.P.offsets['hW/kernel'] == 0) else _f(d, D)
        self.gdot_fresh = False
        if self.dropout:
            in_e, in_d = D + Cn, self.off + L + Cn
            self.u_enc, self.u_dec = _f(d, B, 4, in_e), _f(d, B, 4, in_d)
            self._masks_given = False
            self.xm_e = _f(d, 4, BT, D)
            self.xm_d = torch.zeros(4, BT, self.xz_ld, dtype=torch.float32, device=d)
            self.wm_e, self.wm_d = _f(d, 4, B, Cn), _f(d, 4, B, Cn)
            self.dxg, self.dwg = _f(d, BT, self.xz_ld), _f(d, B, Cn)

    def folds_noise(self):
        return bool((self.fuse_pair or (self.use_mx and self.fuse_latent)) and self.sparse_inputs and self.cfg['D'] % 2 == 0)

    def frames_u8_route(self):
        cfg, B = self.cfg, self.B
        D, H, L, T = cfg['D'], cfg['H'], cfg['L'], cfg['T']
        if not (self.frames_u8 and self.fuse_head and self.bf16_wgrad and self.dense_hw_grad and D % 4 == 0 and self.sparse_inputs
                and ops.dense_outer_bf16_supported(B, T * D, D, T * D, D) and ops.sparse_dense_supported(D)
                and ops.lstm_wgrad_supported(4 * H, D, H, 0, 2) and (not self.off or ops.lstm_wgrad_supported(4 * H, D, H, L, 2))):
            return None
        if self.use_mx:
            return 'gather' if (self.dense_hw_fwd and ops.dense_window_fwd_bf16_supported(B, T * D, D, T * D, D)) else None
        if self.fuse_pair and self.can_stage_in_label():
            return 'label'
        return None

    def frames_u8_supported(self):
        return self.frames_u8_route() is not None

    def forward(self, X, Xp, eps_W, eps_Z, w_true=None, keep_gates=True, nll=None, target=None, noise=None, frames8=None):
        if frames8 is not None and (target is not None or not self.frames_exact_bf16 or not self.frames_u8_supported()):
            raise ValueError("frames8 needs the large-batch path (frames_u8_supported()), frames_exact_bf16 and the input frames as "
                             "the target")
        self._f8 = frames8
        target = X if target is None else target
        cfg, P, B = self.cfg, self.P, self.B
        self._nll_done = False
        self._noise = None
        if noise is not None:
            if self.folds_noise():
                seed, sw, sz, fw, fz, step, step_dev = noise
                self._noise = (ops.noise_draw(seed, sw, fw, step, step_dev), ops.noise_draw(seed, sz, fz, step, step_dev))
            else:
                ops.philox_normal2(eps_W, B * (cfg['C'] - 1), noise[1], noise[3], eps_Z, B * cfg['T'] * cfg['L'], noise[2],
                                   noise[4], noise[0], noise[5], step_dev=noise[6])
        D, H, L, T, Cn = cfg['D'], cfg['H'], cfg['L'], cfg['T'], cfg['C']
        C1, BT, G4 = Cn - 1, B * T, 4 * H
        g, ws = ops.gemm, self.ws
        if cfg['use_x_prev'] and frames8 is None and Xp.data_ptr() != self.XZ.data_ptr():
            self.XZ.view(B, T, self.xz_ld)[:, :, :D].copy_(Xp.view(B, T, D))
        if self.fuse_pair:
            return self._forward_pair(X, eps_W, eps_Z, w_true, nll, target)
        if self.use_mx:
            return self._forward_mx(X, eps_W, eps_Z, w_true, nll, target)
        if self.dropout and self._train_pass:
            if noise is not None:
                row0 = int(noise[3]) // max(cfg['C'] - 1, 1)
                for u, sid in ((self.u_enc, 2), (self.u_dec, 3)):
                    per_row = u.shape[1] * u.shape[2]
                    ops.philox_uniform(u, B * per_row, noise[0], noise[5], sid, row0 * per_row, step_dev=noise[6])
                self._masks_given = True
            elif not self._masks_given:
                raise RuntimeError("training pass with dropout=%g and neither noise=... nor set_dropout_uniforms(): the masks "
                                   "would come from uninitialised memory" % self.dropout)
            return self._forward_dropout(X, eps_W, eps_Z, w_true, nll, target)
        if self.sparse_inputs:
            ops.sparse_proj(BT, D, G4, X, D, P.p('encoder_h/kernel'), self.gates_enc)
        else:
            with self._side():
                g(X, P.p('encoder_h/kernel'), self.gates_enc, BT, G4, D, ws=self.ws2)
        off = self.off
        self._label_forward(X, eps_W, w_true)
        self._join()
        ops.lstm_seq_fwd(B, T, self.gates_enc, self.wk_enc, P.p('encoder_h/recurrent_kernel'), self.hs_enc,
                         self.cs_enc, self.gates_enc, gate_act=self.gate_act, H=H)
        if self.fuse_latent:
            ops.latent_head_fwd(BT, H, L, self.hs_enc, P.p('Zargs/kernel'), P.p('Zargs/bias'), eps_Z, self.zargs, self.Z,
                                self.xz_ld, self.rowkl)
        else:
            g(self.hs_enc, P.p('Zargs/kernel'), self.zargs, BT, 2 * L, H, bias=P.p('Zargs/bias'), ws=ws)
            ops.gauss_fwd(BT, L, self.zargs, eps_Z, self.Z, self.xz_ld, self.rowkl)
        self._join()
        g(self.XZ, P.p('decoder_h/kernel'), self.gates_dec, BT, G4, off + L, lda=self.xz_ld, ws=ws)
        ops.lstm_seq_fwd(B, T, self.gates_dec, self.wk_dec, P.p('decoder_h/recurrent_kernel'), self.hs_dec,
                         self.cs_dec, self.gates_dec, gate_act=self.gate_act, H=H)
        self._output_head(target, nll)

    def _forward_mx(self, X, eps_W, eps_Z, w_true, nll, target):
        cfg, P, B = self.cfg, self.P, self.B
        D, H, L, T = cfg['D'], cfg['H'], cfg['L'], cfg['T']
        BT, off = B * T, self.off
        f8 = self._f8
        if f8 is not None:
            X = f8[0]
        self._label_forward(X, eps_W, w_true)
        ops.lstm_mx_fwd(B, T, X, D, D, P.p('encoder_h/kernel'), None, 0, 0, None, self.wk_enc,
                        P.p('encoder_h/recurrent_kernel'), self.hs_enc, self.gates_enc, self.cs_enc, gate_act=self.gate_act)
        if self.fuse_latent:
            nz = getattr(self, '_noise', None)
            ops.latent_head_fwd(BT, H, L, self.hs_enc, P.p('Zargs/kernel'), P.p('Zargs/bias'), eps_Z, self.zargs, self.Z,
                                self.xz_ld, self.rowkl, noise=nz[1] if nz else None)
        else:
            ops.gemm(self.hs_enc, P.p('Zargs/kernel'), self.zargs, BT, 2 * L, H, bias=P.p('Zargs/bias'), ws=self.ws)
            ops.gauss_fwd(BT, L, self.zargs, eps_Z, self.Z, self.xz_ld, self.rowkl)
        hist, hist_ld = (f8[1], D) if (f8 is not None and off) else (self.XZ if off else None, self.xz_ld)
        ops.lstm_mx_fwd(B, T, hist, hist_ld, off, P.p('decoder_h/kernel') if off else None,
                        self.Z, self.xz_ld, L, P.rows(P.params, 'decoder_h/kernel', off), self.wk_dec,
                        P.p('decoder_h/recurrent_kernel'), self.hs_dec, self.gates_dec, self.cs_dec, gate_act=self.gate_act)
        self._output_head(X if f8 is not None else target, nll)

    def _dense_hw_fwd_now(self):
        cfg = self.cfg
        return self.dense_hw_fwd and self.frames_exact_bf16 and \
            ops.dense_window_fwd_bf16_supported(self.B, cfg['T'] * cfg['D'], cfg['D'], cfg['T'] * cfg['D'], cfg['D'])

    def can_stage_in_label(self):
        return self.fuse_pair and self.sparse_inputs and self.cfg['D'] % 2 == 0 and not self.fuse_notes and \
            not (self.dense_hw_fwd and ops.dense_window_fwd_bf16_supported(self.B, self.cfg['T'] * self.cfg['D'], self.cfg['D'],
                                                                         self.cfg['T'] * self.cfg['D'], self.cfg['D']))

    def _label_forward(self, X, eps_W, w_true, pack=None, stage=None, proj=None):
        cfg, P, B = self.cfg, self.P, self.B
        D, H, L, T, Cn, off = cfg['D'], cfg['H'], cfg['L'], cfg['T'], cfg['C'], self.off
        G4 = 4 * H
        tail = (P.p('Wargs/kernel'), P.p('Wargs/bias'), eps_W, w_true, cfg['w_log_var_prior'],
                P.rows(P.params, 'encoder_h/kernel', D), P.p('encoder_h/bias'),
                P.rows(P.params, 'decoder_h/kernel', off + L), P.p('decoder_h/bias'),
                self.wargs, self.W, self.rowloss, self.wk_enc, self.wk_dec)
        if self.sparse_inputs and D % 2 == 0:
            nz = getattr(self, '_noise', None)
            parts = None
            if stage is None and self._dense_hw_fwd_now():
                if self.ws_hw is None:
                    self.ws_hw = ops.Workspace(self.device)
                parts = ops.dense_window_fwd_bf16(B, T * D, D, X, T * D, P.p('hW/kernel'), D, self.ws_hw)
            ops.vrnn_label_fwd_x(B, D, Cn, G4, X, T * D, T * D, P.p('hW/kernel'), P.p('hW/bias'), self.hW, *tail,
                                 noise=nz[0] if nz else None, pack=pack, parts=parts, stage=stage, proj=proj)
        else:
            ops.gemm(X, P.p('hW/kernel'), self.hW, B, D, T * D, bias=P.p('hW/bias'), act=ACT_RELU, ws=self.ws)
            ops.vrnn_label_fwd(B, D, Cn, G4, self.hW, *tail)

    def _output_head(self, X, nll):
        cfg, P = self.cfg, self.P
        D, H, BT = cfg['D'], cfg['H'], self.B * cfg['T']
        self._head_done = False
        if nll is not None:
            scale, need_grads = nll
            if need_grads and self.fuse_head:
                ops.out_head_train(BT, H, D, self.hs_dec, P.p('X_decoded_mean/kernel'), P.p('X_decoded_mean/bias'), X, scale,
                                   self.rownll, self.dhs, P.g('X_decoded_mean/kernel'), P.g('X_decoded_mean/bias'),
                                   self.ws, logits=self.logits if self.keep_logits else None, defer=self._rq())
                self._head_done = True
            else:
                ops.gemm_bce(self.hs_dec, P.p('X_decoded_mean/kernel'), P.p('X_decoded_mean/bias'), X, scale, self.logits,
                             self.dlogits if need_grads else None, self.rownll, BT, D, H)
            self._nll_done = True
        else:
            ops.gemm(self.hs_dec, P.p('X_decoded_mean/kernel'), self.logits, BT, D, H, bias=P.p('X_decoded_mean/bias'),
                     ws=self.ws)

    def _forward_pair(self, X, eps_W, eps_Z, w_true, nll=None, target=None):
        cfg, P, B = self.cfg, self.P, self.B
        D, H, L, T, Cn = cfg['D'], cfg['H'], cfg['L'], cfg['T'], cfg['C']
        BT, G4, off = B * T, 4 * H, self.off
        g, ws = ops.gemm, self.ws
        pack = (L, P.p('encoder_h/recurrent_kernel'), P.p('decoder_h/recurrent_kernel'),
                P.rows(P.params, 'decoder_h/kernel', off), P.p('Zargs/kernel'), self.pair_pack)
        pack_in_label = self.sparse_inputs and D % 2 == 0
        if not pack_in_label:
            ops.lstm_pair_pack(*pack)
        stage = self.stage_spec if pack_in_label else None
        self.stage_spec = None
        f8 = self._f8
        if f8 is not None and stage is None:
            raise ValueError("frames8 on the pair path: the byte batch is what the label launch's own stage leaves (ops.label_stage)")
        proj = None
        if stage is not None and f8 is not None and self.front_fused and self.sparse_inputs and not self.fuse_notes and \
                ops.vrnn_label_fwd_x_proj_supported(B, D, T * D, T, G4):
            proj = (T, G4, P.p('encoder_h/kernel'), self.gates_enc, P.p('decoder_h/kernel') if off else None,
                    self.gates_dec if off else None)
        if stage is not None:
            self._label_forward(X, eps_W, w_true, pack=pack, stage=stage, proj=proj)
        notes = None
        if proj is not None:
            pass
        elif self.fuse_notes and self.notes_valid:
            notes = (self.notes_enc, P.p('encoder_h/kernel'), self.notes_dec if off else None,
                     P.p('decoder_h/kernel') if off else None)
        elif self.sparse_inputs:
            cur, hist, hist_ld = (X, self.XZ, self.xz_ld) if f8 is None else (f8[0], f8[1], D)
            if off:
                ops.sparse_proj2(BT, G4, (D, cur, D, P.p('encoder_h/kernel'), self.gates_enc),
                                 (off, hist, hist_ld, P.p('decoder_h/kernel'), self.gates_dec))
            else:
                ops.sparse_proj(BT, D, G4, cur, D, P.p('encoder_h/kernel'), self.gates_enc)
        else:
            g(X, P.p('encoder_h/kernel'), self.gates_enc, BT, G4, D, ws=ws)
            if off:
                g(self.XZ, P.p('decoder_h/kernel'), self.gates_dec, BT, G4, off, lda=self.xz_ld, ws=ws)
        if stage is None:
            self._label_forward(X, eps_W, w_true, pack=pack if pack_in_label else None)
        nz = getattr(self, '_noise', None)
        ops.lstm_pair_fwd(B, T, L, self.gates_enc, self.wk_enc, self.gates_dec, off > 0, self.wk_dec, self.pair_pack,
                          P.p('Zargs/bias'), eps_Z, self.hs_enc, self.cs_enc, self.hs_dec, self.cs_dec, self.zargs, self.Z,
                          self.xz_ld, self.klterm, gate_act=self.gate_act, noise=nz[1] if nz else None, notes=notes)
        self._output_head(f8[0] if f8 is not None else (X if target is None else target), nll)

    def xp_view(self):
        return self.XZ.view(self.B, self.cfg['T'], self.xz_ld)[:, :, :self.cfg['D']]

    def x_hat(self):
        cfg, P = self.cfg, self.P
        ops.gemm(self.hs_dec, P.p('X_decoded_mean/kernel'), self.dlogits, self.B * cfg['T'], cfg['D'], cfg['H'],
                 bias=P.p('X_decoded_mean/bias'), act=ACT_SIGMOID, ws=self.ws)
        return self.dlogits

    def _wgrad_args(self, name, X_in, x_ld, x_rows, hs, dz, x8=None):
        cfg, P = self.cfg, self.P
        H, T, L = cfg['H'], cfg['T'], cfg['L']
        nz = L if name == 'decoder_h' else 0
        nx = x_rows - nz
        if not (self.bf16_wgrad and nx > 0 and ops.lstm_wgrad_supported(4 * H, nx, H, nz, self.frames_exact_bf16)):
            return None
        xs, xs_ld = (X_in, x_ld) if (x8 is None or nx == 0) else (x8, nx)
        return (self.B * T, 4 * H, xs, xs_ld, nx, self.frames_exact_bf16, hs, H, H, T, X_in[:, nx:] if nz else None, x_ld, nz,
                dz, P.g(name + '/kernel'), P.g(name + '/recurrent_kernel'),
                P.rows(P.grads, name + '/kernel', nx) if nz else None)

    def _lstm_wgrads(self, name, X_in, x_ld, x_rows, hs, dz, dzsum, w_row, ws, products=True, x8=None):
        cfg, P, B = self.cfg, self.P, self.B
        H, Cn = cfg['H'], cfg['C']
        G4 = 4 * H
        rq = self._rq()
        if products:
# ... 175 lines not shown
```

### classifying-vae-lstm_amd/ops.py

```python
import ctypes as C

import torch

from . import _lib
from ._lib import ACT_NONE, ACT_RELU, ACT_SIGMOID, ACT_MASKPOS, check


def _ptr(t):
    return None if t is None else C.c_void_p(t.data_ptr())


def _stream():
    return C.c_void_p(torch.cuda.current_stream().cuda_stream)


class Workspace:

    def __init__(self, device, nbytes=1 << 20):
        self.device = device
        self.buf = torch.empty(int(nbytes), dtype=torch.uint8, device=device)

    def ensure(self, nbytes):
        if self.buf.numel() < nbytes:
            self.buf = torch.empty(int(nbytes * 1.25) + 256, dtype=torch.uint8, device=self.device)
# ... 76 lines not shown
          "clv_gemm_f32")


def gemm_grouped_tn(probs, N, K, B, ws, ldb=None, beta=0.0, split_k=None, defer=None, split_scale=1):
    L = _lib.lib()
    arr = (_lib.GemmProb * len(probs))()
    for i, p in enumerate(probs):
        A = p.get('A')
        arr[i] = _lib.GemmProb(A.data_ptr() if A is not None else None, p.get('lda', p['M']), p['M'],
                               p['C'].data_ptr(), p.get('ldc', N), p.get('shift', 0), p.get('zero_period', 0),
                               int(p.get('ones', 0)))
    n = len(probs)
    if split_k is None:
        split_k = L.clv_gemm_grouped_auto_split(arr, n, N, K)
        if split_k > 1:
            split_k *= int(split_scale)
    wsp, wsb, job = None, 0, None
    if split_k > 1:
        need = L.clv_gemm_grouped_workspace_bytes(arr, n, N, split_k)
        buf = defer.scratch(need) if defer is not None else ws.ensure(need)
        wsp, wsb = _ptr(buf), buf.numel()
        job = defer.next_job() if defer is not None else None
    check(L.clv_gemm_grouped_tn(arr, n, N, K, _ptr(B), ldb if ldb is not None else N, float(beta), split_k,
                                         wsp, wsb, job, _stream()), "clv_gemm_grouped_tn")


def lstm_wgrad_supported(N, nx, nh, nz, x_exact_bf16):
    return bool(_lib.lib().clv_lstm_wgrad_supported(N, nx, nh, nz, int(bool(x_exact_bf16))))


def lstm_wgrad(K, N, X, ldx, nx, x_exact_bf16, H, ldh, nh, T, Z, ldz, nz, dz, dKx, dU, dKz, ws, defer=None, beta=0.0,
               split_scale=1):
    L = _lib.lib()
    need = L.clv_lstm_wgrad_workspace_bytes(K, N, nx, nh, nz, int(split_scale))
    buf = defer.scratch(need) if defer is not None else ws.ensure(need)
    job = defer.next_job() if defer is not None else None
    check(L.clv_lstm_wgrad(K, N, _ptr(X), ldx, nx, _frames_mode(X, x_exact_bf16), _ptr(H), ldh, nh, 1, T,
                              _ptr(Z), ldz, nz, _ptr(dz), N, _ptr(dKx), N, _ptr(dU), N, _ptr(dKz), N, float(beta),
                              int(split_scale), _ptr(buf), buf.numel(), job, _stream()), "clv_lstm_wgrad")


def _wgrad_problem(K, N, X, ldx, nx, x_exact_bf16, H, ldh, nh, T, Z, ldz, nz, dz, dKx, dU, dKz, beta=0.0):
    w = _lib.WgradProblem()
    w.K, w.N = K, N
    w.X, w.ldx, w.nx, w.x_exact_bf16 = _ptr(X), ldx, nx, _frames_mode(X, x_exact_bf16)
    w.H, w.ldh, w.nh, w.h_shift, w.h_zero_period = _ptr(H), ldh, nh, 1, T
    w.Z, w.ldz, w.nz = _ptr(Z), ldz, nz
    w.dz, w.lddz = _ptr(dz), N
    w.dKx, w.ld_kx, w.dU, w.ld_u, w.dKz, w.ld_kz = _ptr(dKx), N, _ptr(dU), N, _ptr(dKz), N
    w.beta = float(beta)
    return w


def lstm_wgrad_pair_supported(p, q):
    a, b = _wgrad_problem(*p), _wgrad_problem(*q)
    return bool(_lib.lib().clv_lstm_wgrad_pair_supported(C.byref(a), C.byref(b)))


def lstm_wgrad_pair(p, q, ws, defer=None, split_scale=1):
    L = _lib.lib()
    probs, jobs = [], []
    for i, t in enumerate((p, q)):
        w = _wgrad_problem(*t)
        need = L.clv_lstm_wgrad_pair_workspace_bytes(w.K, w.N, w.nx, w.nh, w.nz, int(split_scale))
        buf = defer.scratch(need) if defer is not None else ws[i].ensure(need)
        jobs.append(defer.next_job() if defer is not None else None)
        w.ws, w.ws_bytes = _ptr(buf), buf.numel()
        probs.append(w)
    check(L.clv_lstm_wgrad_pair(C.byref(probs[0]), C.byref(probs[1]), int(split_scale), jobs[0], jobs[1], _stream()),
          "clv_lstm_wgrad_pair")


def gemm_bce(A, B, bias, Y, scale, logits, dlogits, rownll, M, N, K, lda=None, ldb=None, ldy=None, ldc=None):
    check(_lib.lib().clv_gemm_bce_f32(M, N, K, _ptr(A), lda if lda is not None else K, _ptr(B),
                                      ldb if ldb is not None else N, _ptr(bias), _ptr(Y), ldy if ldy is not None else N,
                                      float(scale), _ptr(logits), _ptr(dlogits), ldc if ldc is not None else N,
                                      _ptr(rownll), _stream()), "clv_gemm_bce_f32")


def out_head_train_supported(H, D):
    return bool(_lib.lib().clv_out_head_train_supported(H, D))


def out_head_train(R, H, D, hs, Wo, bo, Y, scale, rownll, dhs, dWo, dbo, ws, logits=None, dlogits=None, ldy=None,
                   defer=None):
    L = _lib.lib()
    need = L.clv_out_head_train_workspace_bytes(R)
    buf = defer.scratch(need) if defer is not None else ws.ensure(need)
    job = defer.next_job() if defer is not None else None
    check(L.clv_out_head_train(R, H, D, _ptr(hs), _ptr(Wo), _ptr(bo), _ptr(Y), _is_u8(Y), ldy if ldy is not None else D,
                               float(scale), _ptr(logits), _ptr(rownll), _ptr(dlogits), _ptr(dhs), _ptr(dWo), _ptr(dbo),
                               _ptr(buf), buf.numel(), job, _stream()), "clv_out_head_train")


def latent_head_supported(H, L):
    return bool(_lib.lib().clv_latent_head_supported(H, L))


def latent_head_fwd(R, H, L, hs, Wz, bz, eps, zargs, Z, ldz, rowkl=None, noise=None):
    check(_lib.lib().clv_latent_head_fwd(R, H, L, _ptr(hs), _ptr(Wz), _ptr(bz), _ptr(eps), _ptr(zargs), _ptr(Z), ldz,
                                         _ptr(rowkl), _noise_ref(noise), _stream()), "clv_latent_head_fwd")


def latent_head_bwd(R, H, L, hs, Wz, zargs, eps, dZ, lddz, kl_scale, dhs, dWz, dbz, ws, dzargs=None, defer=None):
    Lb = _lib.lib()
    need = Lb.clv_latent_head_bwd_workspace_bytes(R, L)
    buf = defer.scratch(need) if defer is not None else ws.ensure(need)
    job = defer.next_job() if defer is not None else None
    check(Lb.clv_latent_head_bwd(R, H, L, _ptr(hs), _ptr(Wz), _ptr(zargs), _ptr(eps), _ptr(dZ), lddz, float(kl_scale),
                                 _ptr(dzargs), _ptr(dhs), _ptr(dWz), _ptr(dbz), _ptr(buf), buf.numel(), job, _stream()),
          "clv_latent_head_bwd")


def _prob_array(probs, N):
    arr = (_lib.GemmProb * len(probs))()
    for i, p in enumerate(probs):
        A = p.get('A')
        arr[i] = _lib.GemmProb(A.data_ptr() if A is not None else None, p.get('lda', p['M']), p['M'],
                               p['C'].data_ptr(), p.get('ldc', N), p.get('shift', 0), p.get('zero_period', 0),
                               int(p.get('ones', 0)))
    return arr


def gemm_grouped_tn_small2(probs0, B0, probs1, B1, N, K, ldb=None):
    a0, a1 = _prob_array(probs0, N), _prob_array(probs1, N)
    check(_lib.lib().clv_gemm_grouped_tn_small2(a0, len(probs0), _ptr(B0), a1, len(probs1), _ptr(B1), N, K,
                                                ldb if ldb is not None else N, _stream()), "clv_gemm_grouped_tn_small2")


def loss_sums(terms, out):
    a = []
    for t, n, st in terms:
        a += [_ptr(t), n, st]
    check(_lib.lib().clv_loss_sums(*a, _ptr(out), _stream()), "clv_loss_sums")


def colsum(X, M, N, out, ws, ldx=None, beta=0.0):
    L = _lib.lib()
    buf = ws.ensure(L.clv_colsum_workspace_bytes(M, N))
    check(L.clv_colsum_f32(M, N, _ptr(X), ldx if ldx is not None else N, float(beta), _ptr(out), _ptr(buf),
                           buf.numel(), _stream()), "clv_colsum_f32")


def lstm_seq_fwd(B, T, xproj, rowbias, U, hs, cs, gates, h0=None, c0=None, hT=None, cT=None, gate_act=0, H=88):
    check(_lib.lib().clv_lstm_seq_fwd(B, T, H, gate_act, _ptr(xproj), _ptr(rowbias), _ptr(U), _ptr(h0), _ptr(c0),
                                      _ptr(hs), _ptr(cs), _ptr(gates), _ptr(hT), _ptr(cT), _stream()),
          "clv_lstm_seq_fwd")


def lstm_seq_bwd_z(B, T, U, dhs, cs, gates_inout, dzsum, Kz, nz, dZ, lddz, c0=None, gate_act=0, H=88):
    check(_lib.lib().clv_lstm_seq_bwd_z(B, T, H, gate_act, _ptr(U), _ptr(dhs), _ptr(cs), _ptr(c0), _ptr(gates_inout),
                                        _ptr(dzsum), _ptr(Kz), nz, _ptr(dZ), lddz, _stream()), "clv_lstm_seq_bwd_z")


def lstm_seq_bwd(B, T, U, dhs, cs, gates_inout, dzsum, c0=None, gate_act=0, H=88):
    check(_lib.lib().clv_lstm_seq_bwd(B, T, H, gate_act, _ptr(U), _ptr(dhs), _ptr(cs), _ptr(c0), _ptr(gates_inout),
                                      _ptr(dzsum), _stream()), "clv_lstm_seq_bwd")


def lstm_mx_supported(B, nx, nz, H=88):
    return bool(_lib.lib().clv_lstm_mx_supported(B, H, nx, nz))


def lstm_mx_fwd(B, T, X, ldx, nx, Kx, Z, ldz, nz, Kz, rowbias, U, hs, coef, aux, gate_act=0, H=88):
    check(_lib.lib().clv_lstm_mx_fwd(B, T, H, gate_act, _ptr(X), _is_u8(X) if X is not None else 0, ldx, nx, _ptr(Kx), _ptr(Z), ldz, nz, _ptr(Kz),
                                     _ptr(rowbias), _ptr(U), _ptr(hs), _ptr(coef), _ptr(aux), _stream()), "clv_lstm_mx_fwd")


def lstm_mx_bwd(B, T, U, dhs, aux, coef_inout, dzsum, Kz=None, nz=0, dZ=None, lddz=0, H=88):
    check(_lib.lib().clv_lstm_mx_bwd(B, T, H, _ptr(U), _ptr(dhs), _ptr(aux), _ptr(coef_inout), _ptr(dzsum), _ptr(Kz), nz,
                                     _ptr(dZ), lddz, _stream()), "clv_lstm_mx_bwd")


def sparse_proj_supported(nx, N):
    return bool(_lib.lib().clv_sparse_proj_supported(nx, N))
# ... 186 lines not shown
    rider = None
    if label is not None:
        if lg is not None:
            if defer is not None:
                lbuf = defer.scratch(need_l)
                lbuf_ptr, ljob = lbuf.data_ptr(), defer.next_job_addr()
            else:
                base = buf if buf is not None else ws.ensure(need_l)
                lbuf_ptr = base.data_ptr() + ((need_h + 255) // 256 * 256 if buf is not None else 0)
        rider = _lib.LabelBwdRider(label['D'], label['C'], _ptr(label['Kenc_w']), _ptr(label['Kdec_w']), _ptr(label['wargs']),
                                   _ptr(label['eps']), _ptr(label['onehot']), _ptr(label['W']), _ptr(label['hW']),
                                   _ptr(label['Ka']), float(label['prior']), float(label['class_weight']),
                                   float(label['w_kl_weight']), float(label['inv_b']), _ptr(label['dwargs']),
                                   _ptr(label['dhW']), _ptr(lg[0]) if lg else None, _ptr(lg[1]) if lg else None,
                                   lbuf_ptr, need_l, ljob)
    check(Lb.clv_lstm_pair_bwd(B, T, H, L, gate_act, float(kl_scale), _ptr(pack), _ptr(Wz),
                                  _ptr(dhs_dec), _ptr(aux_dec), _ptr(aux_enc), _ptr(gates_dec), _ptr(gates_enc),
                                  _ptr(dzsum_dec), _ptr(dzsum_enc), _ptr(zargs), _ptr(eps), _ptr(dzargs),
                                  _ptr(hs), _ptr(dWz), _ptr(dbz), _ptr(buf), nbytes, job,
                                  C.byref(rider) if rider is not None else None, _stream()),
          "clv_lstm_pair_bwd")


def label_fwd(B, Cn, mean, logvar, ld_in, eps, onehot, prior, w, rowloss):
    check(_lib.lib().clv_label_fwd(B, Cn, _ptr(mean), _ptr(logvar), ld_in, _ptr(eps), _ptr(onehot), float(prior),
                                   _ptr(w), _ptr(rowloss), _stream()), "clv_label_fwd")


def label_bwd(B, Cn, mean, logvar, ld_in, eps, onehot, w, dw, prior, class_weight, w_kl_weight, inv_b,
              dmean, dlogvar, ld_out):
    check(_lib.lib().clv_label_bwd(B, Cn, _ptr(mean), _ptr(logvar), ld_in, _ptr(eps), _ptr(onehot), _ptr(w), _ptr(dw),
                                   float(prior), float(class_weight), float(w_kl_weight), float(inv_b),
                                   _ptr(dmean), _ptr(dlogvar), ld_out, _stream()), "clv_label_bwd")


def vrnn_label_fwd(B, D, Cn, G4, hW, Ka, ba, eps, onehot, prior, Kenc_w, benc, Kdec_w, bdec, wargs, W, rowloss, rb_enc,
                   rb_dec):
    check(_lib.lib().clv_vrnn_label_fwd(B, D, Cn, G4, _ptr(hW), _ptr(Ka), _ptr(ba), _ptr(eps), _ptr(onehot),
                                        float(prior), _ptr(Kenc_w), _ptr(benc), _ptr(Kdec_w), _ptr(bdec), _ptr(wargs),
                                        _ptr(W), _ptr(rowloss), _ptr(rb_enc), _ptr(rb_dec), _stream()),
          "clv_vrnn_label_fwd")


def noise_draw(seed, stream, first, step=0, step_dev=None):
    return _lib.NoiseDraw(int(seed), int(first), int(stream), int(step), _ptr(step_dev))


def _is_u8(t):
    if t.dtype == torch.uint8:
        return 1
    if t.dtype != torch.float32:
        raise TypeError("frames must be float32 or uint8, got %s" % t.dtype)
    return 0


def _frames_mode(X, exact):
    return 2 if _is_u8(X) else int(bool(exact))


def _noise_ref(noise):
    return C.byref(noise) if noise is not None else None


def label_stage(cur, hist, idx, row0, cursor, X, Xh, hist_chunk, hist_ld, w_src, w_out, bytes_out=None):
    g = _lib.LabelStage()
    g.cur, g.cur_stride, g.cur_offset, g.cur_table = _ptr(cur[0]), int(cur[1]), int(cur[2]), _ptr(cur[3])
    if hist is not None:
        g.hist, g.hist_stride, g.hist_offset, g.hist_table = _ptr(hist[0]), int(hist[1]), int(hist[2]), _ptr(hist[3])
    g.idx, g.row0 = _ptr(idx), int(row0)
    if cursor is not None:
        g.cursor = _lib.BatchCursor(_ptr(cursor[0]), int(cursor[1]), int(cursor[2]), int(cursor[3]), int(cursor[4]))
    g.X, g.Xh, g.hist_chunk, g.hist_ld = _ptr(X), _ptr(Xh), int(hist_chunk), int(hist_ld)
    g.w_src, g.w_out = _ptr(w_src), _ptr(w_out)
    if bytes_out is not None:
        g.X8, g.Xh8 = _ptr(bytes_out[0]), _ptr(bytes_out[1])
    return g


def vrnn_label_fwd_x_proj_supported(B, D, nx, T, N):
    return bool(_lib.lib().clv_vrnn_label_fwd_x_proj_supported(B, D, nx, T, N))


def vrnn_label_fwd_x(B, D, Cn, G4, X, ldx, nx, Kh, bh, hW_out, Ka, ba, eps, onehot, prior, Kenc_w, benc, Kdec_w, bdec, wargs,
                     W, rowloss, rb_enc, rb_dec, noise=None, pack=None, parts=None, stage=None, proj=None):
    pj = None
    if proj is not None:
        if stage is None or parts is not None:
            raise ValueError("proj rides on a stage (the byte stores it names), not on parts")
        T_, N_, kc, oc, kh, oh = proj
        pj = _lib.FrameProj(int(T_), int(N_), int(N_), _ptr(kc), _ptr(oc), _ptr(kh), _ptr(oh))
    ps = None
    if pack is not None:
        L_, ue, ud, kz, wz, out = pack
        ps = _lib.PairPackSrc(88, int(L_), _ptr(ue), _ptr(ud), _ptr(kz), _ptr(wz), _ptr(out))
    tail = (_ptr(bh), _ptr(hW_out), _ptr(Ka), _ptr(ba), _ptr(eps), _ptr(onehot), float(prior), _ptr(Kenc_w), _ptr(benc),
            _ptr(Kdec_w), _ptr(bdec), _ptr(wargs), _ptr(W), _ptr(rowloss), _ptr(rb_enc), _ptr(rb_dec), _noise_ref(noise),
            C.byref(ps) if ps is not None else None, _stream())
    if parts is not None and stage is None:
        check(_lib.lib().clv_vrnn_label_fwd_parts(B, D, Cn, G4, _ptr(parts[0]), int(parts[1]), *tail), "clv_vrnn_label_fwd_parts")
    else:
        check(_lib.lib().clv_vrnn_label_fwd_x(B, D, Cn, G4, _ptr(X), ldx, nx, _ptr(Kh), C.byref(stage) if stage is not None else None,
                                              *tail[:-1], C.byref(pj) if pj is not None else None, tail[-1]), "clv_vrnn_label_fwd_x")


def dense_window_fwd_bf16_supported(Bn, nx, N, ldx, ldk):
    return bool(_lib.lib().clv_dense_window_fwd_bf16_supported(Bn, nx, N, ldx, ldk))


def dense_window_fwd_bf16(Bn, nx, N, X, ldx, K, ldk, ws):
    L = _lib.lib()
    buf = ws.ensure(L.clv_dense_window_fwd_bf16_workspace_bytes(Bn, nx, N))
    check(L.clv_dense_window_fwd_bf16(Bn, nx, N, _ptr(X), _is_u8(X), ldx, _ptr(K), ldk, _ptr(buf), buf.numel(), _stream()),
          "clv_dense_window_fwd_bf16")
    return buf, L.clv_dense_window_fwd_bf16_splits(Bn, nx)


def vrnn_label_bwd(B, D, Cn, G4, dzsum_enc, dzsum_dec, Kenc_w, Kdec_w, wargs, eps, onehot, W, hW, Ka, prior,
                   class_weight, w_kl_weight, inv_b, dwargs, dhW, layer_grad=None, ws=None, defer=None):
    Lb = _lib.lib()
    dKa, dba, buf, nbytes, job = None, None, None, 0, None
    if layer_grad is not None:
        dKa, dba = layer_grad
        need = Lb.clv_vrnn_label_bwd_workspace_bytes(B, D, Cn)
        buf = defer.scratch(need) if defer is not None else ws.ensure(need)
        nbytes = buf.numel()
        job = defer.next_job() if defer is not None else None
    check(Lb.clv_vrnn_label_bwd(B, D, Cn, G4, _ptr(dzsum_enc), _ptr(dzsum_dec), _ptr(Kenc_w), _ptr(Kdec_w),
                                   _ptr(wargs), _ptr(eps), _ptr(onehot), _ptr(W), _ptr(hW), _ptr(Ka),
                                   float(prior), float(class_weight), float(w_kl_weight), float(inv_b),
                                   _ptr(dwargs), _ptr(dhW), _ptr(dKa), _ptr(dba), _ptr(buf), nbytes, job, _stream()),
          "clv_vrnn_label_bwd")


def gauss_fwd(R, Ld, zargs, eps, z, ldz, rowkl):
    check(_lib.lib().clv_gauss_fwd(R, Ld, _ptr(zargs), _ptr(eps), _ptr(z), ldz, _ptr(rowkl), _stream()),
          "clv_gauss_fwd")


def gauss_bwd(R, Ld, zargs, eps, dz, lddz, kl_scale, dzargs):
    check(_lib.lib().clv_gauss_bwd(R, Ld, _ptr(zargs), _ptr(eps), _ptr(dz), lddz, float(kl_scale), _ptr(dzargs),
                                   _stream()), "clv_gauss_bwd")


def bernoulli_nll(R, D, logits, y, ldy, scale, rownll, dlogits):
    check(_lib.lib().clv_bernoulli_nll(R, D, _ptr(logits), _ptr(y), ldy, float(scale), _ptr(rownll), _ptr(dlogits),
                                       _stream()), "clv_bernoulli_nll")


def sum_strided(n, x, stride, scale, out):
    check(_lib.lib().clv_sum_strided(n, _ptr(x), stride, float(scale), _ptr(out), _stream()), "clv_sum_strided")


def axpy(n, alpha, x, y):
    check(_lib.lib().clv_axpy(n, float(alpha), _ptr(x), _ptr(y), _stream()), "clv_axpy")


def gather_rows(rows, row_elems, src, idx, out, chunk=0, out_ld=0):
    check(_lib.lib().clv_gather_rows(rows, row_elems, _ptr(src), _ptr(idx), _ptr(out), chunk, out_ld, _stream()),
          "clv_gather_rows")


NOTE_ROW, NOTE_NONE = 96, 88


def gather_rows_multi(rows, idx, segs, row0=0, notes=None, cursor=None):
    n = len(segs)
    P, I, U = C.c_void_p * n, C.c_int64 * n, C.c_int32 * n
    src = P(*[s_[0].data_ptr() for s_ in segs])
    if any(s_[1].dtype == torch.uint8 and s_[0].dtype != torch.uint8 for s_ in segs):
        raise TypeError("a uint8 output takes a uint8 source")
    u8 = U(*[(2 if s_[1].dtype == torch.uint8 else 1) if s_[0].dtype == torch.uint8 else 0 for s_ in segs])
    out = P(*[s_[1].data_ptr() for s_ in segs])
    re = I(*[int(s_[2]) for s_ in segs])
    ch = I(*[int(s_[3]) for s_ in segs])
    ld = I(*[int(s_[4]) for s_ in segs])
    ext = [tuple(s_[5:8]) + (0, 0, None)[len(s_[5:8]):] for s_ in segs]
    st = I(*[int(e[0]) for e in ext])
    of = I(*[int(e[1]) for e in ext])
    tb = P(*[(e[2].data_ptr() if e[2] is not None else None) for e in ext])
    nt = P(*[(t.data_ptr() if t is not None else None) for t in (notes or [None] * n)])
    cur = None
    if cursor is not None:
        cur = C.byref(_lib.BatchCursor(cursor[0].data_ptr(), int(cursor[1]), int(cursor[2]), int(cursor[3]), int(cursor[4])))
    check(_lib.lib().clv_gather_rows_multi(rows, _ptr(idx), int(row0), n, src, u8, out, re, ch, ld, st, of, tb, nt, cur, _stream()),
          "clv_gather_rows_multi")
# ... 169 lines not shown
```

### include/clvae.h

```cpp
#ifndef CLVAE_H
#define CLVAE_H

#include <stddef.h>
#include <stdint.h>

#ifdef __cplusplus
extern "C" {
#endif

#define CLV_OK          0
#define CLV_EINVAL     (-1)
#define CLV_EWORKSPACE (-2)
#define CLV_ENOGPU     (-3)

#define CLV_ACT_NONE     0
#define CLV_ACT_RELU     1
#define CLV_ACT_SIGMOID  2
#define CLV_ACT_MASKPOS  3

#define CLV_GATE_HARD_SIGMOID 0
#define CLV_GATE_SIGMOID      1

typedef struct clv_pair_pack_src {
  int H, L;
// ... 209 lines not shown
                  const float* Kx_dec, const float* Kz, const float* Kw_dec, const float* b_dec,
                  const float* U_dec, const float* Wo, const float* bo, const uint8_t* clamp,
                  float inv_temperature, float z_temperature, float* Xs, float* xhat, void* stream);
int clv_vae_vary(int N, int T, int D, int H, int L, int C, int use_x_prev, int hist_source, uint64_t seed,
                 const float* sources, const float* x0, const float* w_enc, const float* w_dec, const float* Kh,
                 const float* bh, const float* Kz, const float* bz, const float* Kd, const float* bd,
                 const float* Ko, const float* bo, const uint8_t* clamp, float inv_temperature,
                 float z_temperature, float* Xs, float* xhat, void* stream);
int clv_take_frame(int64_t n, int T, int D, const float* src, const int32_t* step_dev, float* out, void* stream);

int clv_vrnn_vary_latents(int N, int T, int D, int H, int L, int C, int gate_act, int hist_source, uint64_t seed,
                          const float* sources, const float* x0, const float* w_enc, const float* w_dec,
                          const float* Kx_enc, const float* Kw_enc, const float* b_enc, const float* U_enc,
                          const float* Wz, const float* bz,
                          const float* Kx_dec, const float* Kz, const float* Kw_dec, const float* b_dec,
                          const float* U_dec, const float* Wo, const float* bo, const uint8_t* clamp,
                          float inv_temperature, float z_temperature, float* Xs, float* xhat, float* zout, void* stream);
int clv_vae_vary_latents(int N, int T, int D, int H, int L, int C, int use_x_prev, int hist_source, uint64_t seed,
                         const float* sources, const float* x0, const float* w_enc, const float* w_dec, const float* Kh,
                         const float* bh, const float* Kz, const float* bz, const float* Kd, const float* bd,
                         const float* Ko, const float* bo, const uint8_t* clamp, float inv_temperature,
                         float z_temperature, float* Xs, float* xhat, float* zout, void* stream);
int clv_vrnn_decode(int N, int T, int D, int H, int L, int C, int gate_act, uint64_t seed, const float* z_in,
                    const float* x0, const float* history, const float* w_dec, const int32_t* noise_rows,
                    const float* Kx_dec, const float* Kz, const float* Kw_dec, const float* b_dec,
                    const float* U_dec, const float* Wo, const float* bo, const uint8_t* clamp,
                    float inv_temperature, float* Xs, float* xhat, void* stream);
int clv_vae_decode(int N, int T, int D, int H, int L, int C, int use_x_prev, uint64_t seed, const float* z_in,
                   const float* x0, const float* history, const float* w_dec, const int32_t* noise_rows,
                   const float* Kd, const float* bd, const float* Ko, const float* bo, const uint8_t* clamp,
                   float inv_temperature, float* Xs, float* xhat, void* stream);

int clv_vrnn_generate_resume(int N, int S, int nsteps, int D, int H, int L, int C, int gate_act, int z_prior,
                             uint64_t seed, const float* x_seed, const float* w,
                             const float* Kx_enc, const float* Kw_enc, const float* b_enc, const float* U_enc,
                             const float* Wz, const float* bz,
                             const float* Kx_dec, const float* Kz, const float* Kw_dec, const float* b_dec,
                             const float* U_dec, const float* Wo, const float* bo, const uint8_t* clamp,
                             float inv_temperature, float z_temperature, uint32_t t0, const float* state_in,
                             float* state_out, float* Xs, float* xhat, void* stream);
int clv_vae_generate_resume(int N, int nsteps, int D, int H, int L, int C, int use_x_prev, int z_prior, uint64_t seed,
                            const float* w, const float* Kh, const float* bh, const float* Kz, const float* bz,
                            const float* Kd, const float* bd, const float* Ko, const float* bo, const uint8_t* clamp,
                            float inv_temperature, float z_temperature, uint32_t t0, const float* state_in,
                            float* state_out, float* Xs, float* xhat, void* stream);

int clv_lerp_rows(int64_t R, int64_t n, const float* a, const int32_t* ia, const float* b, const int32_t* ib,
                  const float* alpha, float* out, void* stream);

int clv_label_fwd(int B, int C, const float* mean, const float* logvar, int ld_in,
                  const float* eps, const float* onehot, float prior_logvar,
                  float* w, float* rowloss, void* stream);
int clv_label_bwd(int B, int C, const float* mean, const float* logvar, int ld_in,
                  const float* eps, const float* onehot, const float* w, const float* dw,
                  float prior_logvar, float class_weight, float w_kl_weight, float inv_b,
                  float* dmean, float* dlogvar, int ld_out, void* stream);

int clv_vae_fused_supported(int D, int H, int Hc, int C, int L);
size_t clv_vae_fused_workspace_bytes(int B, int D, int H, int Hc, int C, int L, int use_x_prev);

typedef struct clv_vae_step_opts {
  int draw;
  uint32_t stream_w, stream_z, step;
  uint64_t noise_seed, first_w, first_z;
  const int32_t* step_dev;
  float* loss_means;
  int32_t* bump_iterations;
  int bf16;
} clv_vae_step_opts;

int clv_vrnn_label_fwd(int B, int D, int C, int G4, const float* hW, const float* Ka, const float* ba,
                       const float* eps, const float* onehot, float prior_logvar,
                       const float* Kenc_w, const float* benc, const float* Kdec_w, const float* bdec,
                       float* wargs, float* W, float* rowloss, float* rb_enc, float* rb_dec, void* stream);
int clv_vrnn_label_fwd_x(int B, int D, int C, int G4, const float* X, int ldx, int nx, const float* Kh,
                         const clv_label_stage* stage,
                         const float* bh, float* hW_out, const float* Ka, const float* ba,
                         float* eps, const float* onehot, float prior_logvar,
                         const float* Kenc_w, const float* benc, const float* Kdec_w, const float* bdec,
                         float* wargs, float* W, float* rowloss, float* rb_enc, float* rb_dec,
                         const clv_noise_draw* noise, const clv_pair_pack_src* pack,
                         const clv_frame_proj* proj,
                         void* stream);
int clv_vrnn_label_fwd_x_proj_supported(int B, int D, int nx, int T, int N);
int clv_dense_window_fwd_bf16_supported(int Bn, int nx, int N, int ldx, int ldk);
int clv_dense_window_fwd_bf16_splits(int Bn, int nx);
size_t clv_dense_window_fwd_bf16_workspace_bytes(int Bn, int nx, int N);
int clv_dense_window_fwd_bf16(int Bn, int nx, int N, const void* X, int x_u8, int ldx, const float* K, int ldk, float* part,
                              size_t part_bytes, void* stream);
int clv_vrnn_label_fwd_parts(int B, int D, int C, int G4, const float* part, int splits,
                             const float* bh, float* hW_out, const float* Ka, const float* ba,
                             float* eps, const float* onehot, float prior_logvar,
                             const float* Kenc_w, const float* benc, const float* Kdec_w, const float* bdec,
                             float* wargs, float* W, float* rowloss, float* rb_enc, float* rb_dec,
                             const clv_noise_draw* noise, const clv_pair_pack_src* pack, void* stream);
int clv_vae_fused_step(int B, int D, int H, int Hc, int C, int L, int use_x_prev,
                       const float* x, const float* xp, const float* target, const float* onehot,
                       const clv_label_stage* stage, float* eps_w, float* eps_z,
                       const float* params, const int64_t* host_offsets12, long n_params,
                       float prior_logvar, float class_weight, float kl_weight, float w_kl_weight,
                       int need_grads, float* grads, void* ws, size_t ws_bytes,
                       float* logits, float* w_out, float* wargs_out, float* zargs_out,
                       float* rownll, float* rowkl, float* rowloss, const clv_vae_step_opts* opts, void* stream);
size_t clv_vrnn_label_bwd_workspace_bytes(int B, int D, int C);
int clv_vrnn_label_bwd(int B, int D, int C, int G4, const float* dzsum_enc, const float* dzsum_dec,
                          const float* Kenc_w, const float* Kdec_w, const float* wargs, const float* eps,
                          const float* onehot, const float* W, const float* hW, const float* Ka,
                          float prior_logvar, float class_weight, float w_kl_weight, float inv_b,
                          float* dwargs, float* dhW, float* dKa, float* dba, void* ws, size_t ws_bytes,
                          clv_reduce_job* job, void* stream);

int clv_gauss_fwd(int R, int L, const float* zargs, const float* eps, float* z, int ldz,
                  float* rowkl, void* stream);
int clv_gauss_bwd(int R, int L, const float* zargs, const float* eps, const float* dz, int lddz,
                  float kl_scale, float* dzargs, void* stream);

int clv_bernoulli_nll(int R, int D, const float* logits, const float* y, int ldy, float scale,
                      float* rownll, float* dlogits, void* stream);
int clv_gemm_bce_f32(int M, int N, int K, const float* A, int lda, const float* B, int ldb, const float* bias,
                     const float* Y, int ldy, float scale, float* logits, float* dlogits, int ldc,
                     float* rownll, void* stream);

int clv_out_head_train_supported(int H, int D);
size_t clv_out_head_train_workspace_bytes(int R);
int clv_out_head_train(int R, int H, int D, const float* hs, const float* Wo, const float* bo,
                       const void* Y, int y_u8, int ldy, float scale, float* logits, float* rownll, float* dlogits,
                       float* dhs, float* dWo, float* dbo, void* ws, size_t ws_bytes, clv_reduce_job* job,
                       void* stream);

int clv_latent_head_supported(int H, int L);
size_t clv_latent_head_bwd_workspace_bytes(int R, int L);
int clv_latent_head_fwd(int R, int H, int L, const float* hs, const float* Wz, const float* bz, float* eps,
                        float* zargs, float* Z, int ldz, float* rowkl, const clv_noise_draw* noise, void* stream);
int clv_latent_head_bwd(int R, int H, int L, const float* hs, const float* Wz, const float* zargs, const float* eps,
                        const float* dZ, int lddz, float kl_scale, float* dzargs, float* dhs, float* dWz, float* dbz,
                        void* ws, size_t ws_bytes, clv_reduce_job* job, void* stream);

int clv_act_grad(int64_t n, int act, const float* y, const float* dy, float* dpre, void* stream);
int clv_axpy(int64_t n, float alpha, const float* x, float* y, void* stream);

int clv_sparse_proj_supported(int nx, int N);
size_t clv_sparse_proj_lds_bytes(int nx, int N);
int clv_sparse_proj(int R, int nx, int N, const void* X, int x_u8, int ldx, const float* K, float* out, int ldo, void* stream);
int clv_sparse_proj2(int R, int N, int ldo, int x_u8, int nx0, const void* X0, int ldx0, const float* K0, float* out0,
                     int nx1, const void* X1, int ldx1, const float* K1, float* out1, void* stream);

int clv_sparse_dense_supported(int N);
int clv_sparse_dense(int R, int nx, int N, const float* X, int ldx, const float* K, const float* bias, int act,
                     float* out, int ldo, void* stream);
int clv_sparse_outer(int Bn, int nx, int N, const float* X, int ldx, const float* G, int ldg, float* out, int ldo,
                        float* colsum, const float* Hact, int ldh, const float* hbias, float* gdot, void* stream);

int clv_dense_outer_bf16_supported(int Bn, int nx, int N, int ldx, int ldg);
int clv_dense_outer_bf16(int Bn, int nx, int N, const void* X, int x_u8, int ldx, const float* G, int ldg, float* out, int ldo,
                         float* colsum, const float* Hact, int ldh, const float* hbias, float* gdot, void* stream);

int clv_gather_rows(int64_t rows, int64_t row_elems, const float* src, const int64_t* idx, float* out,
                    int64_t chunk, int64_t out_ld, void* stream);
#define CLV_NOTE_ROW 96
#define CLV_NOTE_NONE 88
int clv_gather_rows_multi(int64_t rows, const int64_t* idx, int64_t row0, int nseg,
                                 const void* const* src, const int32_t* src_u8, float* const* out,
                                 const int64_t* row_elems, const int64_t* chunk, const int64_t* out_ld,
                                 const int64_t* src_stride, const int64_t* src_offset,
                                 const int64_t* const* src_table, unsigned char* const* notes_out,
                                 const clv_batch_cursor* cursor, void* stream);

int clv_loss_sums(const float* x0, int n0, int s0, const float* x1, int n1, int s1, const float* x2, int n2, int s2,
                  const float* x3, int n3, int s3, const float* x4, int n4, int s4, float* out, void* stream);

int clv_sum_strided(int n, const float* x, int stride, float scale, float* out, void* stream);

typedef struct clv_param_desc {
  int64_t offset;
  int32_t rows;
  int32_t cols;
  int64_t col_offset;
  int32_t is_matrix;
  int32_t pad_;
} clv_param_desc;
size_t clv_adam_wn_plan_bytes(const clv_param_desc* host_table, int n_tensors);
int clv_adam_wn_plan_build(const clv_param_desc* host_table, int n_tensors, void* host_blob);
size_t clv_adam_wn_workspace_bytes(const clv_param_desc* host_table, int n_tensors);
#define CLV_STEP_ADVANCED (-2)
#define CLV_OPT_ADAM     0
#define CLV_OPT_ADAM_WN  1
#define CLV_OPT_RMSPROP  2
typedef struct clv_adam_known_sums {
  int tensor;
  int use;
  const float* gdot;
  float* vnorm2;
} clv_adam_known_sums;
int clv_adam_wn_step(const clv_param_desc* host_table, int n_tensors, const void* plan_dev,
                        float* params, const float* grads, float* m, float* v,
                        float* mg, float* vg, float* s,
                        int32_t* iterations_dev, int step_t, float lr, float beta1, float beta2, float eps,
                        int weightnorm, const clv_adam_known_sums* known, void* ws, size_t ws_bytes, void* stream);

int clv_philox_normal(float* out, int64_t n, uint64_t seed, uint32_t step, const int32_t* step_dev,
                      uint32_t stream_id, uint64_t first_index, void* stream);
int clv_philox_uniform(float* out, int64_t n, uint64_t seed, uint32_t step, const int32_t* step_dev,
                       uint32_t stream_id, uint64_t first_index, void* stream);
int clv_philox_normal2(float* out0, int64_t n0, uint32_t stream_id0, uint64_t first_index0,
                       float* out1, int64_t n1, uint32_t stream_id1, uint64_t first_index1,
                       uint64_t seed, uint32_t step, const int32_t* step_dev, void* stream);
int clv_i32_add(int32_t* counter, int32_t v, void* stream);
int clv_bernoulli_sample(int64_t n, const float* p, const float* u, float* x, void* stream);
int clv_bernoulli_sample_clamped(int64_t n, int D, int nsteps, int S, const float* p, const float* u, const uint8_t* clamp,
                                 const int32_t* step_dev, float* x, void* stream);
int clv_dropout_rows(int R, int T, int n, const float* X, int ldx, const float* U, int ldu, float rate, float beta,
// ... 49 lines not shown
```

Baseline: 102.6 million timesteps/s.

## Precompute output-head weight images inside the label forward kernel

Adds a pass that writes pre-packed (likely bf16 fragment) images of the output head weights Wo/bo. That pass is folded into the early label-forward kernel, spare threads do the conversion, and the later out_head_train kernel reads the ready images instead of repacking the weights every call. A freshness flag ensures the images are only used when they were produced in the same step. In exchange the label kernel does extra work, and a register cap (amdgpu_num_sgpr) is added to the parts kernel, which could cause spills.

After: 101.1 million timesteps/s. 0.985x the previous value.

```diff
diff --git a/classifying-vae-lstm_amd/_lib.py b/classifying-vae-lstm_amd/_lib.py
--- a/classifying-vae-lstm_amd/_lib.py
+++ b/classifying-vae-lstm_amd/_lib.py
@@ -162,6 +162,9 @@
     "clv_out_head_train_supported": (_i, [_i, _i]),
     "clv_out_head_train_workspace_bytes": (_sz, [_i]),
     "clv_out_head_train": (_i, [_i, _i, _i, _p, _p, _p, _p, _i, _i, _f, _p, _p, _p, _p, _p, _p, _p, _sz, _p, _p]),
+    "clv_out_head_train_img": (_i, [_i, _i, _i, _p, _p, _p, _p, _i, _i, _f, _p, _p, _p, _p, _p, _p, _p, _sz, _p, _p, _p]),
+    "clv_out_head_images_bytes": (_sz, []),
+    "clv_out_head_images": (_i, [_p, _p, _p, _p]),
     "clv_latent_head_supported": (_i, [_i, _i]),
     "clv_latent_head_bwd_workspace_bytes": (_sz, [_i, _i]),
     "clv_latent_head_fwd": (_i, [_i, _i, _i, _p, _p, _p, _p, _p, _p, _i, _p, _p, _p]),
@@ -195,9 +198,13 @@
     "clv_vrnn_label_fwd": (_i, [_i, _i, _i, _i, _p, _p, _p, _p, _p, _f, _p, _p, _p, _p, _p, _p, _p, _p, _p, _p]),
     "clv_vrnn_label_fwd_x": (_i, [_i, _i, _i, _i, _p, _i, _i, _p, _p, _p, _p, _p, _p, _p, _p, _f, _p, _p, _p, _p, _p, _p, _p, _p, _p,
                                   _p, _p, _p, _p]),
+    "clv_vrnn_label_fwd_x_oimg": (_i, [_i, _i, _i, _i, _p, _i, _i, _p, _p, _p, _p, _p, _p, _p, _p, _f, _p, _p, _p, _p, _p, _p, _p, _p, _p,
+                                       _p, _p, _p, _p, _p, _p, _p]),
     "clv_vrnn_label_fwd_x_proj_supported": (_i, [_i, _i, _i, _i, _i]),
     "clv_vrnn_label_fwd_parts": (_i, [_i, _i, _i, _i, _p, _i, _p, _p, _p, _p, _p, _p, _f, _p, _p, _p, _p, _p, _p, _p, _p, _p,
                                   _p, _p, _p]),
+    "clv_vrnn_label_fwd_parts_oimg": (_i, [_i, _i, _i, _i, _p, _i, _p, _p, _p, _p, _p, _p, _f, _p, _p, _p, _p, _p, _p, _p, _p, _p,
+                                           _p, _p, _p, _p, _p, _p]),
     "clv_dense_window_fwd_bf16_supported": (_i, [_i, _i, _i, _i, _i]),
     "clv_dense_window_fwd_bf16_splits": (_i, [_i, _i]),
     "clv_dense_window_fwd_bf16_workspace_bytes": (_sz, [_i, _i, _i]),
diff --git a/classifying-vae-lstm_amd/csrc/label_head.hip b/classifying-vae-lstm_amd/csrc/label_head.hip
--- a/classifying-vae-lstm_amd/csrc/label_head.hip
+++ b/classifying-vae-lstm_amd/csrc/label_head.hip
@@ -3,6 +3,7 @@
 #include "philox.h"
 #include "reduce_job.h"
 #include "label_bwd_row.h"
+#include "out_head_images.h"
 
 namespace clv {
 
@@ -143,6 +144,7 @@
   const float* bh;
   int nx, ldx;
   PairPackArgs pack;
+  OutHeadImagesArgs oimg;
   const float* part; int splits;
   struct Stage {
     int on;
@@ -155,6 +157,7 @@
     unsigned char* X8; unsigned char* Xh8;
   } stage;
 };
+template <bool OIMG>
 __device__ __forceinline__ void label_fwd_x_block(const LabelFwdXArgs& ax, const int b, float2 (*part)[64], float* s_h, float* s_wargs,
                                                   float* s_w) {
   const LabelFwdArgs& a = ax.l;
@@ -164,6 +167,7 @@
       ax.pack.out[i] = pair_pack_element(i, ax.pack.L, ax.pack.U_e, ax.pack.U_d, ax.pack.Kz, ax.pack.Wz,
                                          [](const float* p) { return *p; });
   }
+  if (OIMG && ax.oimg.out) ob_images_write(ax.oimg, b * 1024 + tid, a.B * 1024);
   const int wave = __builtin_amdgcn_readfirstlane(tid >> 6);
   const int n2 = a.D / 2;
   const int lc = min(lane, n2 - 1);
@@ -259,10 +263,11 @@
   label_fwd_row<1024>(a, b, tid, s_h, s_wargs, s_w, oh_row);
 }
 
+template <bool OIMG>
 __global__ __launch_bounds__(1024) void vrnn_label_fwd_x_kernel(LabelFwdXArgs ax) {
   __shared__ float2 part[16][64];
   __shared__ float s_h[128], s_wargs[2 * LH_MAXC], s_w[LH_MAXC];
-  label_fwd_x_block(ax, (int)blockIdx.x, part, s_h, s_wargs, s_w);
+  label_fwd_x_block<OIMG>(ax, (int)blockIdx.x, part, s_h, s_wargs, s_w);
 }
 
 constexpr int FP_RMAX = 64;
@@ -448,12 +453,12 @@
   __shared__ const unsigned char* rowp[FP_RMAX];
   extern __shared__ __attribute__((aligned(16))) float fp_kl[];
   FRONT_STAMP(0);
-  if ((int)blockIdx.x < ax.l.B) label_fwd_x_block(ax, (int)blockIdx.x, part, s_h, s_wargs, s_w);
+  if ((int)blockIdx.x < ax.l.B) label_fwd_x_block<true>(ax, (int)blockIdx.x, part, s_h, s_wargs, s_w);
   else frame_proj_block(ax, fp, (int)blockIdx.x - ax.l.B, fp_kl, rowp);
   FRONT_STAMP(1);
 }
 
-__global__ __launch_bounds__(LH_T) void vrnn_label_fwd_parts_kernel(LabelFwdXArgs ax) {
+__global__ __launch_bounds__(LH_T) __attribute__((amdgpu_num_sgpr(82))) void vrnn_label_fwd_parts_kernel(LabelFwdXArgs ax) {
   constexpr int NWV = LH_T / 64;
   __shared__ float2 part[NWV][64];
   __shared__ float s_h[128], s_wargs[2 * LH_MAXC], s_w[LH_MAXC];
@@ -464,6 +469,7 @@
       ax.pack.out[i] = pair_pack_element(i, ax.pack.L, ax.pack.U_e, ax.pack.U_d, ax.pack.Kz, ax.pack.Wz,
                                          [](const float* p) { return *p; });
   }
+  if (ax.oimg.out) ob_images_write(ax.oimg, (int)(blockIdx.x * LH_T + tid), (int)(gridDim.x * LH_T));
   const int wave = __builtin_amdgcn_readfirstlane(tid >> 6);
   const int b = blockIdx.x;
   const int n2 = a.D / 2;
@@ -564,7 +570,10 @@
                               float* eps, const float* onehot, float prior_logvar,
                               const float* Kenc_w, const float* benc, const float* Kdec_w, const float* bdec,
                               float* wargs, float* W, float* rowloss, float* rb_enc, float* rb_dec,
-                              const clv_noise_draw* noise, const clv_pair_pack_src* pack, const clv_frame_proj* proj, void* stream) {
+                              const clv_noise_draw* noise, const clv_pair_pack_src* pack, const clv_frame_proj* proj,
+                              const float* head_Wo, const float* head_bo, void* wo_images, void* stream) {
+  const bool oimg = wo_images != nullptr;
+  if (oimg && (!head_Wo || !head_bo || ((uintptr_t)head_Wo) % 16 || ((uintptr_t)wo_images) % 16)) return CLV_EINVAL;
   if (pack && (pack->H != LH || !clv_lstm_pair_supported(pack->H, pack->L) || !pack->U_enc || !pack->U_dec || !pack->Kz ||
                !pack->Wz || !pack->pack || ((uintptr_t)pack->pack) % 16))
     return CLV_EINVAL;
@@ -590,7 +599,7 @@
       !rb_enc || !rb_dec)
     return CLV_EINVAL;
   LabelFwdXArgs a{{B, D, C, G4, hW_out, Ka, ba, eps, {0, 0, 0, 0, 0, 0, nullptr}, onehot, prior_logvar, Kenc_w, benc, Kdec_w, bdec,
-                   wargs, W, rowloss, rb_enc, rb_dec}, X, Kh, bh, nx, ldx, {0, nullptr, nullptr, nullptr, nullptr, nullptr}, part, splits, {}};
+                   wargs, W, rowloss, rb_enc, rb_dec}, X, Kh, bh, nx, ldx, {0, nullptr, nullptr, nullptr, nullptr, nullptr}, {nullptr, nullptr, nullptr}, part, splits, {}};
   if (stage) {
     const clv_label_stage& g = *stage;
     a.stage = LabelFwdXArgs::Stage{1, g.cur, g.hist, (long long)g.cur_stride, (long long)g.cur_offset, (long long)g.hist_stride,
@@ -601,6 +610,7 @@
     if (g.w_src) a.l.onehot = g.w_src;
   }
   if (pack) a.pack = PairPackArgs{pack->L, pack->U_enc, pack->U_dec, pack->Kz, pack->Wz, reinterpret_cast<float4*>(pack->pack)};
+  if (oimg) a.oimg = OutHeadImagesArgs{head_Wo, head_bo, (char*)wo_images};
   if (noise) {
     a.l.noise.on = 1; a.l.noise.k0 = (uint32_t)noise->seed; a.l.noise.k1 = (uint32_t)(noise->seed >> 32);
     a.l.noise.stream = noise->stream; a.l.noise.step = noise->step; a.l.noise.first = noise->first;
@@ -634,7 +644,8 @@
   }
   ProfScope p("vrnn_label_fwd", s);
   if (part) hipLaunchKernelGGL(vrnn_label_fwd_parts_kernel, dim3(B), dim3(LH_T), 0, s, a);
-  else hipLaunchKernelGGL(vrnn_label_fwd_x_kernel, dim3(B), dim3(1024), 0, s, a);
+  else if (oimg) hipLaunchKernelGGL(vrnn_label_fwd_x_kernel<true>, dim3(B), dim3(1024), 0, s, a);
+  else hipLaunchKernelGGL(vrnn_label_fwd_x_kernel<false>, dim3(B), dim3(1024), 0, s, a);
   return launch_status();
 }
 
@@ -647,6 +658,22 @@
 extern "C" int clv_vrnn_label_fwd_x_proj_supported(int B, int D, int nx, int T, int N) {
   return B >= 1 && D >= 4 && D <= 128 && D % 4 == 0 && T >= 1 && (long long)T * D == nx && N >= 8 && N % 8 == 0 && N / 2 <= 64 * clv::FP_NC &&
          (size_t)D * (N / 2) * sizeof(float) <= 64 * 1024 && (size_t)B * T * N * sizeof(float) < ((size_t)1 << 31);
+}
+
+extern "C" int clv_vrnn_label_fwd_x_oimg(int B, int D, int C, int G4, const float* X, int ldx, int nx, const float* Kh,
+                                    const clv_label_stage* stage,
+                                    const float* bh, float* hW_out, const float* Ka, const float* ba,
+                                    float* eps, const float* onehot, float prior_logvar,
+                                    const float* Kenc_w, const float* benc, const float* Kdec_w, const float* bdec,
+                                    float* wargs, float* W, float* rowloss, float* rb_enc, float* rb_dec,
+                                    const clv_noise_draw* noise, const clv_pair_pack_src* pack, const clv_frame_proj* proj,
+                                    const float* head_Wo, const float* head_bo, void* wo_images, void* stream) {
+  if (stage)
+    return label_fwd_x_launch(B, D, C, G4, stage->X, ldx, nx, Kh, nullptr, 0, stage, bh, hW_out, Ka, ba, eps, stage->w_src,
+                              prior_logvar, Kenc_w, benc, Kdec_w, bdec, wargs, W, rowloss, rb_enc, rb_dec, noise, pack, proj, head_Wo, head_bo, wo_images, stream);
+  if (proj) return CLV_EINVAL;
+  return label_fwd_x_launch(B, D, C, G4, X, ldx, nx, Kh, nullptr, 0, nullptr, bh, hW_out, Ka, ba, eps, onehot, prior_logvar, Kenc_w, benc,
+                            Kdec_w, bdec, wargs, W, rowloss, rb_enc, rb_dec, noise, pack, nullptr, head_Wo, head_bo, wo_images, stream);
 }
 
 extern "C" int clv_vrnn_label_fwd_x(int B, int D, int C, int G4, const float* X, int ldx, int nx, const float* Kh,
@@ -657,12 +684,20 @@
                                     float* wargs, float* W, float* rowloss, float* rb_enc, float* rb_dec,
                                     const clv_noise_draw* noise, const clv_pair_pack_src* pack, const clv_frame_proj* proj,
                                     void* stream) {
-  if (stage)
-    return label_fwd_x_launch(B, D, C, G4, stage->X, ldx, nx, Kh, nullptr, 0, stage, bh, hW_out, Ka, ba, eps, stage->w_src,
-                              prior_logvar, Kenc_w, benc, Kdec_w, bdec, wargs, W, rowloss, rb_enc, rb_dec, noise, pack, proj, stream);
-  if (proj) return CLV_EINVAL;
-  return label_fwd_x_launch(B, D, C, G4, X, ldx, nx, Kh, nullptr, 0, nullptr, bh, hW_out, Ka, ba, eps, onehot, prior_logvar, Kenc_w, benc,
-                            Kdec_w, bdec, wargs, W, rowloss, rb_enc, rb_dec, noise, pack, nullptr, stream);
+  return clv_vrnn_label_fwd_x_oimg(B, D, C, G4, X, ldx, nx, Kh, stage, bh, hW_out, Ka, ba, eps, onehot, prior_logvar, Kenc_w, benc, Kdec_w,
+                                   bdec, wargs, W, rowloss, rb_enc, rb_dec, noise, pack, proj, nullptr, nullptr, nullptr, stream);
+}
+
+extern "C" int clv_vrnn_label_fwd_parts_oimg(int B, int D, int C, int G4, const float* part, int splits,
+                                        const float* bh, float* hW_out, const float* Ka, const float* ba,
+                                        float* eps, const float* onehot, float prior_logvar,
+                                        const float* Kenc_w, const float* benc, const float* Kdec_w, const float* bdec,
+                                        float* wargs, float* W, float* rowloss, float* rb_enc, float* rb_dec,
+                                        const clv_noise_draw* noise, const clv_pair_pack_src* pack,
+                                        const float* head_Wo, const float* head_bo, void* wo_images, void* stream) {
+  if (!part) return CLV_EINVAL;
+  return label_fwd_x_launch(B, D, C, G4, nullptr, 0, 0, nullptr, part, splits, nullptr, bh, hW_out, Ka, ba, eps, onehot, prior_logvar, Kenc_w,
+                            benc, Kdec_w, bdec, wargs, W, rowloss, rb_enc, rb_dec, noise, pack, nullptr, head_Wo, head_bo, wo_images, stream);
 }
 
 extern "C" int clv_vrnn_label_fwd_parts(int B, int D, int C, int G4, const float* part, int splits,
@@ -671,7 +706,6 @@
                                         const float* Kenc_w, const float* benc, const float* Kdec_w, const float* bdec,
                                         float* wargs, float* W, float* rowloss, float* rb_enc, float* rb_dec,
                                         const clv_noise_draw* noise, const clv_pair_pack_src* pack, void* stream) {
-  if (!part) return CLV_EINVAL;
-  return label_fwd_x_launch(B, D, C, G4, nullptr, 0, 0, nullptr, part, splits, nullptr, bh, hW_out, Ka, ba, eps, onehot, prior_logvar, Kenc_w,
-                            benc, Kdec_w, bdec, wargs, W, rowloss, rb_enc, rb_dec, noise, pack, nullptr, stream);
-}
+  return clv_vrnn_label_fwd_parts_oimg(B, D, C, G4, part, splits, bh, hW_out, Ka, ba, eps, onehot, prior_logvar, Kenc_w, benc, Kdec_w, bdec,
+                                       wargs, W, rowloss, rb_enc, rb_dec, noise, pack, nullptr, nullptr, nullptr, stream);
+}
diff --git a/classifying-vae-lstm_amd/csrc/out_head.hip b/classifying-vae-lstm_amd/csrc/out_head.hip
--- a/classifying-vae-lstm_amd/csrc/out_head.hip
+++ b/classifying-vae-lstm_amd/csrc/out_head.hip
@@ -1,4 +1,5 @@
 #include "out_head_args.h"
+#include "out_head_images.h"
 #include "reduce_job.h"
 
 namespace clv {
@@ -267,24 +268,41 @@
 
 extern "C" int clv_out_head_train_supported(int H, int D) { return H == clv::OH && D == clv::OH; }
 
+namespace clv {
+__global__ __launch_bounds__(256) void out_head_images_kernel(OutHeadImagesArgs a) {
+  ob_images_write(a, (int)(blockIdx.x * 256 + threadIdx.x), (int)(gridDim.x * 256));
+}
+}
+
+extern "C" size_t clv_out_head_images_bytes(void) { return (size_t)2 * clv::OB_IMG; }
+
+extern "C" int clv_out_head_images(const float* Wo, const float* bo, void* images, void* stream) {
+  using namespace clv;
+  if (!Wo || !bo || !images || ((uintptr_t)Wo) % 16 != 0 || ((uintptr_t)images) % 16 != 0) return CLV_EINVAL;
+  ProfScope p("out_head_images", (hipStream_t)stream);
+  hipLaunchKernelGGL(out_head_images_kernel, dim3(OB_IMAGE_ITEMS / 256), dim3(256), 0, (hipStream_t)stream,
+                     OutHeadImagesArgs{Wo, bo, (char*)images});
+  return launch_status();
+}
+
 extern "C" size_t clv_out_head_train_workspace_bytes(int R) {
   return R > 0 ? (size_t)clv::out_head_wgs(R) * clv::OH_SLAB_ROWS * clv::OH * sizeof(float) : 0;
 }
 
-extern "C" int clv_out_head_train(int R, int H, int D, const float* hs, const float* Wo, const float* bo,
+extern "C" int clv_out_head_train_img(int R, int H, int D, const float* hs, const float* Wo, const float* bo,
                                   const void* Y, int y_u8, int ldy, float scale, float* logits, float* rownll, float* dlogits,
                                   float* dhs, float* dWo, float* dbo, void* ws, size_t ws_bytes, clv_reduce_job* job,
-                                  void* stream) {
+                                  const void* wo_images, void* stream) {
   using namespace clv;
   if (!clv_out_head_train_supported(H, D) || R <= 0 || ldy < D) return CLV_EINVAL;
   if (!hs || !Wo || !bo || !Y || !rownll || !dhs || !dWo || !dbo) return CLV_EINVAL;
-  if (((uintptr_t)hs) % 16 != 0 || ((uintptr_t)Wo) % 16 != 0) return CLV_EINVAL;
+  if (((uintptr_t)hs) % 16 != 0 || ((uintptr_t)Wo) % 16 != 0 || ((uintptr_t)wo_images) % 16 != 0) return CLV_EINVAL;
   if (!ws || ws_bytes < clv_out_head_train_workspace_bytes(R)) return CLV_EWORKSPACE;
   hipStream_t s = (hipStream_t)stream;
   const size_t lds = (size_t)(OH * OH_LD + 2 * OH_NW * OH_TILE) * sizeof(float);
   if (int e = clv::allow_dynamic_lds(reinterpret_cast<const void*>(out_head_train_kernel), (int)lds)) return e;
   const int wgs = out_head_wgs(R);
-  OutHeadArgs a{R, ldy, scale, hs, Wo, bo, Y, y_u8 != 0, logits, rownll, dlogits, dhs, (float*)ws};
+  OutHeadArgs a{R, ldy, scale, hs, Wo, bo, Y, y_u8 != 0, logits, rownll, dlogits, dhs, (float*)ws, wo_images};
   static const bool f32_only = [] { const char* e = getenv("CLV_OUT_HEAD_F32"); return e && e[0] == '1'; }();
   if (!(f32_only && !y_u8) && out_head_bf16_ok(a)) {
     if (int e = launch_out_head_bf16(a, wgs, s)) return e;
@@ -308,3 +326,11 @@
   if (job) memset(job, 0, sizeof(*job));
   return launch_reduce(j, s);
 }
+
+extern "C" int clv_out_head_train(int R, int H, int D, const float* hs, const float* Wo, const float* bo,
+                                  const void* Y, int y_u8, int ldy, float scale, float* logits, float* rownll, float* dlogits,
+                                  float* dhs, float* dWo, float* dbo, void* ws, size_t ws_bytes, clv_reduce_job* job,
+                                  void* stream) {
+  return clv_out_head_train_img(R, H, D, hs, Wo, bo, Y, y_u8, ldy, scale, logits, rownll, dlogits, dhs, dWo, dbo, ws, ws_bytes, job,
+                                nullptr, stream);
+}
diff --git a/classifying-vae-lstm_amd/csrc/out_head_args.h b/classifying-vae-lstm_amd/csrc/out_head_args.h
--- a/classifying-vae-lstm_amd/csrc/out_head_args.h
+++ b/classifying-vae-lstm_amd/csrc/out_head_args.h
@@ -6,6 +6,8 @@
 constexpr int OH = 88;
 constexpr int OH_SLAB_ROWS = OH + 1;
 constexpr int OH_RB = 128;
+constexpr int OB_FRAG = 1024;
+constexpr int OB_IMG = 3 * 6 * 3 * OB_FRAG;
 
 struct OutHeadArgs {
   int R, ldy;
@@ -20,6 +22,7 @@
   float* dlogits;
   float* dhs;
   float* partial;
+  const void* images;
 };
 
 bool out_head_bf16_ok(const OutHeadArgs& a);
diff --git a/classifying-vae-lstm_amd/csrc/out_head_bf16.hip b/classifying-vae-lstm_amd/csrc/out_head_bf16.hip
--- a/classifying-vae-lstm_amd/csrc/out_head_bf16.hip
+++ b/classifying-vae-lstm_amd/csrc/out_head_bf16.hip
@@ -8,8 +8,6 @@
 typedef unsigned u32x4 __attribute__((ext_vector_type(4)));
 
 constexpr int OB_NW = 8;
-constexpr int OB_FRAG = 1024;
-constexpr int OB_IMG = 3 * 6 * 3 * OB_FRAG;
 constexpr int OB_DLT = 96 * 16;
 constexpr int OB_LDS = 2 * OB_IMG + OB_NW * OB_DLT * 4;
 static_assert(OB_LDS <= 160 * 1024, "LDS");
@@ -107,7 +105,16 @@
   };
   load_hv(blockIdx.x * OH_RB + wave * 16);
 
-  {
+  if (a.images) {
+    constexpr int NV = 2 * OB_IMG / 16, PT = (NV + 64 * OB_NW - 1) / (64 * OB_NW);
+    const u32x4* src = reinterpret_cast<const u32x4*>(a.images);
+    u32x4 iv[PT];
+#pragma unroll
+    for (int k = 0; k < PT; ++k) iv[k] = src[min(tid + 64 * OB_NW * k, NV - 1)];
+#pragma unroll
+    for (int k = 0; k < PT; ++k)
+      if (tid + 64 * OB_NW * k < NV) reinterpret_cast<u32x4*>(ob_lds)[tid + 64 * OB_NW * k] = iv[k];
+  } else {
     const ob_rsrc_t r_wo = ob_rsrc(a.Wo, (size_t)OH * OH * 4), r_bo = ob_rsrc(a.bo, (size_t)OH * 4);
     const int m = r, qq = q;
     const unsigned l0 = (8 * qq * OH + m) * 4u;
@@ -350,7 +357,7 @@
   auto al = [](const void* p) { return ((uintptr_t)p) % 16 == 0; };
   const size_t widest = (size_t)a.R * (size_t)(a.ldy > OH ? a.ldy : OH) * 4;
   const bool y_ok = a.y_u8 ? (((uintptr_t)a.Y) % 4 == 0) : al(a.Y);
-  return widest < 0x80000000ull && al(a.hs) && y_ok && a.ldy % 4 == 0 && al(a.dhs) && al(a.logits) && al(a.dlogits);
+  return widest < 0x80000000ull && al(a.hs) && y_ok && a.ldy % 4 == 0 && al(a.dhs) && al(a.logits) && al(a.dlogits) && al(a.images);
 }
 
 int launch_out_head_bf16(const OutHeadArgs& a, int wgs, hipStream_t s) {
diff --git a/classifying-vae-lstm_amd/csrc/out_head_images.h b/classifying-vae-lstm_amd/csrc/out_head_images.h
--- /dev/null
+++ b/classifying-vae-lstm_amd/csrc/out_head_images.h
@@ -0,0 +1,54 @@
+#pragma once
+#include "out_head_args.h"
+
+namespace clv {
+
+struct OutHeadImagesArgs {
+  const float* Wo;
+  const float* bo;
+  char* out;
+};
+constexpr int OB_IMAGE_ITEMS = 2 * 18 * 64;
+
+__device__ __forceinline__ void ob_image_item(const OutHeadImagesArgs& a, int i) {
+  typedef unsigned img_u32x4 __attribute__((ext_vector_type(4)));
+  const int F = i >> 6, lane = i & 63, m = lane & 15, qq = lane >> 4;
+  const int img = F >= 18, fr = F - 18 * img, j = fr / 3, s = fr - 3 * j;
+  float v[8];
+  if (!img) {
+    const int note = 16 * j + m, nc = min(note, OH - 1), h0 = 32 * s + 8 * qq;
+    const float* col = a.Wo + min(h0, OH - 8) * OH + nc;
+    const bool ok = h0 < OH && note < OH;
+#pragma unroll
+    for (int e = 0; e < 8; ++e) v[e] = col[e * OH];
+#pragma unroll
+    for (int e = 0; e < 8; ++e) v[e] = ok ? v[e] : 0.f;
+    const float bias = a.bo[nc];
+    if (s == 2 && qq == 3) v[0] = note < OH ? bias : 0.f;
+  } else {
+    const int h = 16 * j + m, n0 = 32 * s + 4 * qq, n1 = n0 + 16;
+    const float* row = a.Wo + min(h, OH - 1) * OH;
+    const float4 lo = *reinterpret_cast<const float4*>(row + n0);
+    const float4 hi = *reinterpret_cast<const float4*>(row + min(n1, OH - 4));
+    const bool okl = h < OH, okh = h < OH && n1 < OH;
+    v[0] = okl ? lo.x : 0.f; v[1] = okl ? lo.y : 0.f; v[2] = okl ? lo.z : 0.f; v[3] = okl ? lo.w : 0.f;
+    v[4] = okh ? hi.x : 0.f; v[5] = okh ? hi.y : 0.f; v[6] = okh ? hi.z : 0.f; v[7] = okh ? hi.w : 0.f;
+  }
+  img_u32x4 f[3];
+#pragma unroll
+  for (int k = 0; k < 4; ++k) {
+    unsigned pc[3];
+    bf16_split_pair_dot2(v[2 * k], v[2 * k + 1], pc);
+    f[0][k] = pc[0]; f[1][k] = pc[1]; f[2][k] = pc[2];
+  }
+  char* base = a.out + img * OB_IMG + fr * OB_FRAG + lane * 16;
+#pragma unroll
+  for (int p = 0; p < 3; ++p) *reinterpret_cast<img_u32x4*>(base + p * 18 * OB_FRAG) = f[p];
+}
+
+__device__ __forceinline__ void ob_images_write(const OutHeadImagesArgs& a, int t, int nthreads) {
+#pragma unroll 1
+  for (int i = t; i < OB_IMAGE_ITEMS; i += nthreads) ob_image_item(a, i);
+}
+
+}
diff --git a/classifying-vae-lstm_amd/engine.py b/classifying-vae-lstm_amd/engine.py
--- a/classifying-vae-lstm_amd/engine.py
+++ b/classifying-vae-lstm_amd/engine.py
@@ -59,6 +59,7 @@
     'frames_u8':      ('CLV_FRAMES_U8',        True,  "the large-batch step widens its byte batch to float (rounds 4-5) instead of reading bytes"),
     'front_fused':    ('CLV_FRONT_FUSED',      True,  "the frame projections as a launch of their own behind the label launch instead of workgroups of it (csrc/label_head.hip: vrnn_front_kernel)"),
     'tail_launch':    ('CLV_TAIL_LAUNCH',      True,  "the hW kernel gradient as a launch of its own in front of grads_tail() instead of workgroups of the reduction launch that ends it (csrc/tail_launch.hip)"),
+    'out_head_images': ('CLV_OUT_HEAD_IMAGES', True, "every workgroup of the fused output head splits Wo into its bf16 piece images itself instead of copying the pair the label forward launch wrote (csrc/out_head_images.h)"),
     'fine_grid':      ('CLV_FINE_GRID',        False, "twice the workgroups, half the rows each, for the LSTM kernel gradients (what tune_dp_schedule may pick next to an all-reduce)"),
     'fuse_notes':     ('CLV_FUSE_NOTES',       False, "input projections gathered inside the pair forward from note lists (+48 us on MI355X: profiles/r03_notes_fusion_ab.txt)"),
 }
@@ -344,6 +345,9 @@
         self.sparse_inputs = sw('sparse_inputs') and ops.sparse_proj_supported(D, 4 * H)
         self.fuse_head = sw('fuse_head') and ops.out_head_train_supported(H, D)
         self._head_done = False
+        self.out_head_images = sw('out_head_images') and self.fuse_head
+        self.wo_images = torch.empty(ops.out_head_images_bytes(), dtype=torch.uint8, device=d) if self.out_head_images else None
+        self._wo_images_fresh = False
         self.keep_logits = sw('keep_logits')
         self.bf16_wgrad = sw('bf16_wgrad')
         self.frames_exact_bf16 = bool(cfg.get('frames_exact_bf16', False))
@@ -430,6 +434,8 @@
             raise ValueError("frames8 needs the large-batch path (frames_u8_supported()), frames_exact_bf16 and the input frames as "
                              "the target")
         self._f8 = frames8
+        self._wo_images_fresh = False
+        self._head_next = nll is not None and bool(nll[1]) and self.fuse_head
         target = X if target is None else target
         cfg, P, B = self.cfg, self.P, self.B
         self._nll_done = False
@@ -531,8 +537,12 @@
                 if self.ws_hw is None:
                     self.ws_hw = ops.Workspace(self.device)
                 parts = ops.dense_window_fwd_bf16(B, T * D, D, X, T * D, P.p('hW/kernel'), D, self.ws_hw)
+            oimg = None
+            if self.out_head_images and getattr(self, '_head_next', False) and (proj is not None or parts is not None or B <= 256):
+                oimg = (P.p('X_decoded_mean/kernel'), P.p('X_decoded_mean/bias'), self.wo_images)
             ops.vrnn_label_fwd_x(B, D, Cn, G4, X, T * D, T * D, P.p('hW/kernel'), P.p('hW/bias'), self.hW, *tail,
-                                 noise=nz[0] if nz else None, pack=pack, parts=parts, stage=stage, proj=proj)
+                                 noise=nz[0] if nz else None, pack=pack, parts=parts, stage=stage, proj=proj, oimg=oimg)
+            self._wo_images_fresh = oimg is not None
         else:
             ops.gemm(X, P.p('hW/kernel'), self.hW, B, D, T * D, bias=P.p('hW/bias'), act=ACT_RELU, ws=self.ws)
             ops.vrnn_label_fwd(B, D, Cn, G4, self.hW, *tail)
@@ -546,7 +556,9 @@
             if need_grads and self.fuse_head:
                 ops.out_head_train(BT, H, D, self.hs_dec, P.p('X_decoded_mean/kernel'), P.p('X_decoded_mean/bias'), X, scale,
                                    self.rownll, self.dhs, P.g('X_decoded_mean/kernel'), P.g('X_decoded_mean/bias'),
-                                   self.ws, logits=self.logits if self.keep_logits else None, defer=self._rq())
+                                   self.ws, logits=self.logits if self.keep_logits else None, defer=self._rq(),
+                                   images=self.wo_images if self._wo_images_fresh else None)
+                self._wo_images_fresh = False
                 self._head_done = True
             else:
                 ops.gemm_bce(self.hs_dec, P.p('X_decoded_mean/kernel'), P.p('X_decoded_mean/bias'), X, scale, self.logits,
diff --git a/classifying-vae-lstm_amd/ops.py b/classifying-vae-lstm_amd/ops.py
--- a/classifying-vae-lstm_amd/ops.py
+++ b/classifying-vae-lstm_amd/ops.py
@@ -182,15 +182,23 @@
     return bool(_lib.lib().clv_out_head_train_supported(H, D))
 
 
+def out_head_images_bytes():
+    return int(_lib.lib().clv_out_head_images_bytes())
+
+
+def out_head_images(Wo, bo, images):
+    check(_lib.lib().clv_out_head_images(_ptr(Wo), _ptr(bo), _ptr(images), _stream()), "clv_out_head_images")
+
+
 def out_head_train(R, H, D, hs, Wo, bo, Y, scale, rownll, dhs, dWo, dbo, ws, logits=None, dlogits=None, ldy=None,
-                   defer=None):
+                   defer=None, images=None):
     L = _lib.lib()
     need = L.clv_out_head_train_workspace_bytes(R)
     buf = defer.scratch(need) if defer is not None else ws.ensure(need)
     job = defer.next_job() if defer is not None else None
-    check(L.clv_out_head_train(R, H, D, _ptr(hs), _ptr(Wo), _ptr(bo), _ptr(Y), _is_u8(Y), ldy if ldy is not None else D,
-                               float(scale), _ptr(logits), _ptr(rownll), _ptr(dlogits), _ptr(dhs), _ptr(dWo), _ptr(dbo),
-                               _ptr(buf), buf.numel(), job, _stream()), "clv_out_head_train")
+    check(L.clv_out_head_train_img(R, H, D, _ptr(hs), _ptr(Wo), _ptr(bo), _ptr(Y), _is_u8(Y), ldy if ldy is not None else D,
+                                   float(scale), _ptr(logits), _ptr(rownll), _ptr(dlogits), _ptr(dhs), _ptr(dWo), _ptr(dbo),
+                                   _ptr(buf), buf.numel(), job, _ptr(images), _stream()), "clv_out_head_train")
 
 
 def latent_head_supported(H, L):
@@ -543,7 +551,7 @@
 
 
 def vrnn_label_fwd_x(B, D, Cn, G4, X, ldx, nx, Kh, bh, hW_out, Ka, ba, eps, onehot, prior, Kenc_w, benc, Kdec_w, bdec, wargs,
-                     W, rowloss, rb_enc, rb_dec, noise=None, pack=None, parts=None, stage=None, proj=None):
+                     W, rowloss, rb_enc, rb_dec, noise=None, pack=None, parts=None, stage=None, proj=None, oimg=None):
     pj = None
     if proj is not None:
         if stage is None or parts is not None:
@@ -556,12 +564,14 @@
         ps = _lib.PairPackSrc(88, int(L_), _ptr(ue), _ptr(ud), _ptr(kz), _ptr(wz), _ptr(out))
     tail = (_ptr(bh), _ptr(hW_out), _ptr(Ka), _ptr(ba), _ptr(eps), _ptr(onehot), float(prior), _ptr(Kenc_w), _ptr(benc),
             _ptr(Kdec_w), _ptr(bdec), _ptr(wargs), _ptr(W), _ptr(rowloss), _ptr(rb_enc), _ptr(rb_dec), _noise_ref(noise),
-            C.byref(ps) if ps is not None else None, _stream())
+            C.byref(ps) if ps is not None else None)
+    last = (*((_ptr(t) for t in oimg) if oimg is not None else (None, None, None)), _stream())
     if parts is not None and stage is None:
-        check(_lib.lib().clv_vrnn_label_fwd_parts(B, D, Cn, G4, _ptr(parts[0]), int(parts[1]), *tail), "clv_vrnn_label_fwd_parts")
+        check(_lib.lib().clv_vrnn_label_fwd_parts_oimg(B, D, Cn, G4, _ptr(parts[0]), int(parts[1]), *tail, *last),
+              "clv_vrnn_label_fwd_parts")
     else:
-        check(_lib.lib().clv_vrnn_label_fwd_x(B, D, Cn, G4, _ptr(X), ldx, nx, _ptr(Kh), C.byref(stage) if stage is not None else None,
-                                              *tail[:-1], C.byref(pj) if pj is not None else None, tail[-1]), "clv_vrnn_label_fwd_x")
+        check(_lib.lib().clv_vrnn_label_fwd_x_oimg(B, D, Cn, G4, _ptr(X), ldx, nx, _ptr(Kh), C.byref(stage) if stage is not None else None,
+                                                   *tail, C.byref(pj) if pj is not None else None, *last), "clv_vrnn_label_fwd_x")
 
 
 def dense_window_fwd_bf16_supported(Bn, nx, N, ldx, ldk):
diff --git a/include/clvae.h b/include/clvae.h
--- a/include/clvae.h
+++ b/include/clvae.h
@@ -315,6 +315,14 @@
                          const clv_noise_draw* noise, const clv_pair_pack_src* pack,
                          const clv_frame_proj* proj,
                          void* stream);
+int clv_vrnn_label_fwd_x_oimg(int B, int D, int C, int G4, const float* X, int ldx, int nx, const float* Kh,
+                              const clv_label_stage* stage,
+                              const float* bh, float* hW_out, const float* Ka, const float* ba,
+                              float* eps, const float* onehot, float prior_logvar,
+                              const float* Kenc_w, const float* benc, const float* Kdec_w, const float* bdec,
+                              float* wargs, float* W, float* rowloss, float* rb_enc, float* rb_dec,
+                              const clv_noise_draw* noise, const clv_pair_pack_src* pack, const clv_frame_proj* proj,
+                              const float* head_Wo, const float* head_bo, void* wo_images, void* stream);
 int clv_vrnn_label_fwd_x_proj_supported(int B, int D, int nx, int T, int N);
 int clv_dense_window_fwd_bf16_supported(int Bn, int nx, int N, int ldx, int ldk);
 int clv_dense_window_fwd_bf16_splits(int Bn, int nx);
@@ -327,6 +335,13 @@
                              const float* Kenc_w, const float* benc, const float* Kdec_w, const float* bdec,
                              float* wargs, float* W, float* rowloss, float* rb_enc, float* rb_dec,
                              const clv_noise_draw* noise, const clv_pair_pack_src* pack, void* stream);
+int clv_vrnn_label_fwd_parts_oimg(int B, int D, int C, int G4, const float* part, int splits,
+                                  const float* bh, float* hW_out, const float* Ka, const float* ba,
+                                  float* eps, const float* onehot, float prior_logvar,
+                                  const float* Kenc_w, const float* benc, const float* Kdec_w, const float* bdec,
+                                  float* wargs, float* W, float* rowloss, float* rb_enc, float* rb_dec,
+                                  const clv_noise_draw* noise, const clv_pair_pack_src* pack,
+                                  const float* head_Wo, const float* head_bo, void* wo_images, void* stream);
 int clv_vae_fused_step(int B, int D, int H, int Hc, int C, int L, int use_x_prev,
                        const float* x, const float* xp, const float* target, const float* onehot,
                        const clv_label_stage* stage, float* eps_w, float* eps_z,
@@ -355,11 +370,17 @@
                      float* rownll, void* stream);
 
 int clv_out_head_train_supported(int H, int D);
+size_t clv_out_head_images_bytes(void);
+int clv_out_head_images(const float* Wo, const float* bo, void* images, void* stream);
 size_t clv_out_head_train_workspace_bytes(int R);
 int clv_out_head_train(int R, int H, int D, const float* hs, const float* Wo, const float* bo,
                        const void* Y, int y_u8, int ldy, float scale, float* logits, float* rownll, float* dlogits,
                        float* dhs, float* dWo, float* dbo, void* ws, size_t ws_bytes, clv_reduce_job* job,
                        void* stream);
+int clv_out_head_train_img(int R, int H, int D, const float* hs, const float* Wo, const float* bo,
+                           const void* Y, int y_u8, int ldy, float scale, float* logits, float* rownll, float* dlogits,
+                           float* dhs, float* dWo, float* dbo, void* ws, size_t ws_bytes, clv_reduce_job* job,
+                           const void* wo_images, void* stream);
 
 int clv_latent_head_supported(int H, int L);
 size_t clv_latent_head_bwd_workspace_bytes(int R, int L);
```
